# SamShue/EKF_SLAM

Measured on AMD Instinct MI355X. Metric: EKF update-steps/sec at N landmarks; HBM GB/s on (I−KH)P vs roofline, higher is better.
Workload: dtype f64

## Files before the change

### ekf_slam_amd/_lib.py

```python
import ctypes
import os
import subprocess

_HERE = os.path.dirname(os.path.abspath(__file__))
LIB_PATH = os.environ.get("EKF_LIB_PATH") or os.path.join(_HERE, "libekfslam.so")

EKF_OK = 0
EKF_ERR_INVALID_ARG, EKF_ERR_NO_DEVICE, EKF_ERR_HIP, EKF_ERR_CAPACITY = 1, 2, 3, 4
EKF_ERR_INDEX, EKF_ERR_LOOKUP, EKF_ERR_STATE, EKF_ERR_COMM = 5, 6, 7, 8
EKF_MODE_KNOWN, EKF_MODE_UC = 0, 1
EKF_COMM_ID_BYTES = 128
EKF_MERGE_BATCH_MAX = 32
EKF_STORE_F64, EKF_STORE_F32 = 0, 1
EKF_ARITH_F64, EKF_ARITH_F32, EKF_ARITH_SPLIT3 = 0, 1, 2
(EKF_KERNEL_DOWNDATE, EKF_KERNEL_GATHER, EKF_KERNEL_PREDICT, EKF_KERNEL_ASSOCIATE, EKF_KERNEL_APPEND,
 EKF_KERNEL_ROWPANEL, EKF_KERNEL_EXCHANGE, EKF_KERNEL_COMPACT, EKF_KERNEL_COUNT) = range(9)

_d = ctypes.c_double
_dp = ctypes.POINTER(ctypes.c_double)
_i32 = ctypes.c_int32
_i64 = ctypes.c_int64
_vp = ctypes.c_void_p


class EkfConfig(ctypes.Structure):
    _fields_ = [("C", _d), ("Rc", _d * 2), ("s_cost", _d), ("s_thresh", _d), ("w_pos", _d),
                ("capacity_landmarks", _i64), ("mode", _i32), ("storage", _i32), ("device", _i32),
                ("tile", _i32), ("rank", _i32), ("world", _i32), ("batch", _i32), ("async_flush", _i32), ("device_assoc", _i32),
                ("pass_direction", _i32), ("force_sharded", _i32), ("pass_arith", _i32), ("reserved", _i32 * 2)]


SIGNATURES = {
    "ekf_abi_version": (_i32, []),
    "ekf_status_string": (ctypes.c_char_p, [_i32]),
    "ekf_config_default": (_i32, [ctypes.POINTER(EkfConfig), _i32]),
    "ekf_create": (_i32, [ctypes.POINTER(EkfConfig), ctypes.POINTER(_vp)]),
    "ekf_destroy": (_i32, [_vp]),
    "ekf_last_error": (ctypes.c_char_p, [_vp]),
    "ekf_set_stream": (_i32, [_vp, _vp]),
    "ekf_sync": (_i32, [_vp]),
    "ekf_flush": (_i32, [_vp]),
    "ekf_pending": (_i32, [_vp, ctypes.POINTER(_i32)]),
    "ekf_set_params": (_i32, [_vp, _d, _dp, _d, _d, _d]),
    "ekf_predict": (_i32, [_vp, _dp]),
    "ekf_motion_model": (_i32, [_dp, _i64, _dp, _dp, _dp]),
    "ekf_append": (_i32, [_vp, _dp, _dp, _dp, _d]),
    "ekf_correct": (_i32, [_vp, _dp, _dp, _i64]),
    "ekf_associate": (_i32, [_vp, _dp, _dp, ctypes.POINTER(_i32), ctypes.POINTER(_i64), _dp, _dp]),
    "ekf_associate_begin": (_i32, [_vp, _dp, _dp, _i32]),
    "ekf_associate_finish": (_i32, [_vp, ctypes.POINTER(_i32), ctypes.POINTER(_i64), _dp, _dp]),
    "ekf_measure": (_i32, [_vp, _dp, _i64, _dp, _dp, _dp, _i64]),
    "ekf_comm_unique_id": (_i32, [ctypes.c_char_p]),
    "ekf_comm_init": (_i32, [_vp, ctypes.c_char_p]),
    "ekf_hint_next": (_i32, [_vp, _i64]),
    "ekf_correct_begin": (_i32, [_vp, _dp, _dp, _i64]),
    "ekf_correct_finish": (_i32, [_vp]),
    "ekf_prefetch_rows": (_i32, [_vp, ctypes.POINTER(_i64), _i32]),
    "ekf_prefetch_next": (_i32, [_vp, ctypes.POINTER(_i64), _i32]),
    "ekf_prefetch_begin": (_i32, [_vp, ctypes.POINTER(_i64), _i32]),
    "ekf_prefetch_finish": (_i32, [_vp]),
    "ekf_exchange_info": (_i32, [_vp, ctypes.POINTER(_vp), ctypes.POINTER(_vp), ctypes.POINTER(_i64),
                                 ctypes.POINTER(_i64)]),
    "ekf_exchange_set_buffers": (_i32, [_vp, _vp, _vp]),
    "ekf_exchange_local": (_i32, [ctypes.POINTER(_vp), _i32]),
    "ekf_exchange_set_hook": (_i32, [_vp, _vp, _vp]),
    "ekf_shard_owner": (_i32, [_i32, _i64, _i64]),
    "ekf_shard_slot": (_i64, [_i32, _i64, _i64]),
    "ekf_shard_panel_source": (_i32, [_i32, _i64, _i64, ctypes.POINTER(_i32), ctypes.POINTER(_i64)]),
    "ekf_num_landmarks": (_i32, [_vp, ctypes.POINTER(_i64)]),
    "ekf_get_x": (_i32, [_vp, _dp]),
    "ekf_set_x": (_i32, [_vp, _dp, _i64]),
    "ekf_get_s": (_i32, [_vp, _dp]),
    "ekf_set_s": (_i32, [_vp, _dp, _i64]),
    "ekf_remove_landmarks": (_i32, [_vp, ctypes.POINTER(_i64), _i64]),
    "ekf_constrain_landmarks": (_i32, [_vp, _i64, _i64, _dp, _dp]),
    "ekf_merge_landmarks": (_i32, [_vp, _i64, _i64, _dp]),
    "ekf_merge_landmarks_batch": (_i32, [_vp, ctypes.POINTER(_i64), ctypes.POINTER(_i64), _i64, _dp, _dp]),
    "ekf_landmark_distance": (_i32, [_vp, _i64, _i64, _dp, _dp, _dp, _dp]),
    "ekf_nearest_landmarks": (_i32, [_vp, _dp, _dp, ctypes.POINTER(_i64)]),
    "ekf_diag_poke_device_signature": (_i32, [_vp, _i64, _d]),
    "ekf_get_P": (_i32, [_vp, _dp]),
    "ekf_set_P": (_i32, [_vp, _dp, _i64]),
    "ekf_get_P_block": (_i32, [_vp, _i64, _i64, _i64, _i64, _dp]),
    "ekf_get_P_diag_blocks": (_i32, [_vp, _dp]),
    "ekf_get_Q": (_i32, [_vp, _dp]),
    "ekf_load_lowrank_state": (_i32, [_vp, _i64, _dp, _dp, _dp, _dp, _i64]),
    "ekf_checkpoint_save": (_i32, [_vp, ctypes.c_char_p]),
    "ekf_checkpoint_load": (_i32, [_vp, ctypes.c_char_p]),
    "ekf_P_digest": (_i32, [_vp, _dp]),
    "ekf_device_bytes": (_i32, [_vp, ctypes.POINTER(_i64)]),
    "ekf_kernel_timing_enable": (_i32, [_vp, _i32, _i32]),
    "ekf_kernel_timing_read": (_i32, [_vp, _i32, ctypes.POINTER(_i64), _dp]),
    "ekf_downdate_kernel_name": (ctypes.c_char_p, [_vp, ctypes.POINTER(_i32)]),
    "ekf_downdate_algorithmic_bytes": (_i32, [_vp, ctypes.POINTER(_i64)]),
}

_LIB = None


class EkfError(RuntimeError):
    def __init__(self, status, message):
        super().__init__("libekfslam status %d: %s" % (status, message))
        self.status = status


def build():
    subprocess.check_call(["make", "-s", "-C", os.path.join(_HERE, "csrc")])


def lib():
    global _LIB
    if _LIB is None:
        if not os.path.exists(LIB_PATH):
            raise ImportError("libekfslam.so is not built (%s); run __graft_entry__.build() or "
                              "`make -C ekf_slam_amd/csrc` -- there is no fallback path" % LIB_PATH)
        if os.environ.get("EKF_NO_TORCH", "0") != "1":
            try:
                import torch
            except ImportError:
                pass
        L = ctypes.CDLL(LIB_PATH)
        for name, (res, args) in SIGNATURES.items():
            fn = getattr(L, name)
            fn.restype = res
            fn.argtypes = args
        _LIB = L
    return _LIB

EXCHANGE_HOOK = ctypes.CFUNCTYPE(ctypes.c_int32, ctypes.c_void_p)
```

### ekf_slam_amd/csrc/gather.h

```cpp
#pragma once

constexpr int kGatherCols = 256;
constexpr int kGatherBlock = kGatherCols + 3 * 64;

__device__ __forceinline__ double lane_bcast(double v, int src) {
    const int lo = __builtin_amdgcn_readlane(__double2loint(v), src), hi = __builtin_amdgcn_readlane(__double2hiint(v), src);
    return __hiloint2double(hi, lo);
}
__device__ __forceinline__ double lane_gather(double v, int src) {
    const int lo = __builtin_amdgcn_ds_bpermute(src << 2, __double2loint(v)), hi = __builtin_amdgcn_ds_bpermute(src << 2, __double2hiint(v));
    return __hiloint2double(hi, lo);
}
__device__ __forceinline__ double lane_xor1(double v) {
    const int lo = __builtin_amdgcn_mov_dpp(__double2loint(v), 0xB1, 0xF, 0xF, true), hi = __builtin_amdgcn_mov_dpp(__double2hiint(v), 0xB1, 0xF, 0xF, true);
    return __hiloint2double(hi, lo);
}
__device__ __forceinline__ void wave_lds_sync() { asm volatile("s_waitcnt lgkmcnt(0)" ::: "memory"); }

constexpr int kFuseMaxRows = 48;
constexpr int kFuseElems = kFuseMaxRows * kFuseMaxRows / 256;

template <typename TS>
__device__ __forceinline__ void gather_decided_other(const DevState &st, const CorrectArgs &a, const DevLoopArgs &dl, int64_t Nd,
                                                     bool append) {
    __shared__ double oa_ll[kGatherCols / 64];
    __shared__ int oa_ix[kGatherCols / 64];
    const int tid = threadIdx.x;
    if (tid >= kGatherCols) return;
    const int cur = a.cur;
    const double *__restrict__ x = st.x[cur];
    const double *__restrict__ strip = st.strip[cur];
    const double *__restrict__ prr = st.prr[cur];
    double *__restrict__ x_nxt = st.x[cur ^ 1];
    double *__restrict__ strip_nxt = st.strip[cur ^ 1];
    double *__restrict__ prr_nxt = st.prr[cur ^ 1];
    const double *__restrict__ dg = st.diag[st.dcur];
    double *__restrict__ dgn = st.diag[st.dcur ^ 1];
    TS *__restrict__ tiles = (TS *)st.tiles;
    const int64_t ldm = st.ldm;
    const int64_t n_old = 2 * Nd, n_new = append ? n_old + 2 : n_old;
    const int64_t c = (int64_t)blockIdx.x * kGatherCols + tid;
    const bool live = c < n_new;
    double pose[3], pr[9];
#pragma unroll
    for (int i = 0; i < 3; ++i) pose[i] = x[i];
#pragma unroll
    for (int i = 0; i < 9; ++i) pr[i] = prr[i];
    double jxr[2][3];
    append_jxr(dl.u0, pose[2], jxr);
    double xn = 0.0, t0 = 0.0, t1 = 0.0, t2 = 0.0, dgc = 0.0, dgl = 0.0;
    if (c < n_old) {
        t0 = strip[c]; t1 = strip[ldm + c]; t2 = strip[2 * ldm + c];
        xn = x[3 + c];
        const double *__restrict__ d = dg + 3 * (c >> 1);
        if (c & 1) { dgl = d[1]; dgc = d[2]; } else dgc = d[0];
        if (append)
            for (int i = 0; i < 2; ++i)
                if (st.tm.mine((n_old + i) >> st.tm.shift, c >> st.tm.shift))
                    pmm_low_store<TS>(tiles, st.tm, n_old + i, c, append_row_entry(jxr, i, t0, t1, t2));
    } else if (live) {
        const int b = (int)(c - n_old);
        const volatile double *loc = dl.loc + 3 * (Nd - dl.loc_base);
        double cblk[3], iblk[3][2];
        append_blocks(jxr, pr, dl.u0, dl.u1, a.R00, a.R01, a.R10, a.R11, cblk, iblk);
        xn = loc[b];
        t0 = iblk[0][b]; t1 = iblk[1][b]; t2 = iblk[2][b];
        const bool own = st.tm.mine(n_old >> st.tm.shift, n_old >> st.tm.shift);
        if (b == 0) {
            dgc = cblk[0];
            if (own) pmm_low_store<TS>(tiles, st.tm, n_old, n_old, cblk[0]);
            st.s[Nd] = (double)(Nd + 1);
        } else {
            dgl = cblk[1]; dgc = cblk[2];
            if (own) { pmm_low_store<TS>(tiles, st.tm, n_old + 1, n_old, cblk[1]); pmm_low_store<TS>(tiles, st.tm, n_old + 1, n_old + 1, cblk[2]); }
        }
    }
    if (live) {
        x_nxt[3 + c] = xn;
        strip_nxt[c] = t0; strip_nxt[ldm + c] = t1; strip_nxt[2 * ldm + c] = t2;
        double *__restrict__ d = dgn + 3 * (c >> 1);
        if (c & 1) { d[1] = dgl; d[2] = dgc; } else d[0] = dgc;
    }
    if (c < st.tm.padded(n_new)) {
        const int64_t out_off = (int64_t)ring_slot(a.pstart, a.npend, st.pcap) * st.pair_stride;
        reinterpret_cast<double2 *>(st.Gp + out_off)[c] = make_double2(0.0, 0.0);
        reinterpret_cast<double2 *>(st.Kp + out_off)[c] = make_double2(0.0, 0.0);
        if (st.Gp32) {
            st.Gp32[out_off + c] = 0.0f; st.Gp32[out_off + ldm + c] = 0.0f;
            st.Kp32[out_off + c] = -0.0f; st.Kp32[out_off + ldm + c] = -0.0f;
        }
    }
    if (blockIdx.x == 0) {
        if (tid < 9) prr_nxt[tid] = prr[tid];
        if (tid < 3) x_nxt[tid] = x[tid];
        if (tid == 0) *dl.dn_out = n_new >> 1;
    }
    if (dl.parts_out == nullptr) return;
    const bool odd = (c & 1) != 0;
    const double xn_o = lane_xor1(xn), t0_o = lane_xor1(t0), t1_o = lane_xor1(t1), t2_o = lane_xor1(t2),
                 d10 = lane_xor1(dgl), d11 = lane_xor1(dgc);
    double ll = INFINITY;
    int64_t ix = INT64_MAX;
    if (live && !odd) {
        const int64_t k = c >> 1;
        double q[24];
#pragma unroll
        for (int i = 0; i < 9; ++i) q[i] = pr[i];
        q[9] = t0; q[10] = t0_o; q[11] = t1; q[12] = t1_o; q[13] = t2; q[14] = t2_o;
        q[15] = dgc; q[16] = d10; q[17] = d10; q[18] = d11;
        q[19] = pose[0]; q[20] = pose[1]; q[21] = pose[2];
        q[22] = xn; q[23] = xn_o;
        SmallSolve so;
        solve_small(q, dl.z0, dl.z1, dl.R00, dl.R01, dl.R10, dl.R11, so);
        const double n0 = so.nu[0], n1 = so.nu[1];
        const double pc = (n0 * so.Phi[0] + n1 * so.Phi[2]) * n0 + (n0 * so.Phi[1] + n1 * so.Phi[3]) * n1;
        const double sk = k == Nd ? (double)(Nd + 1) : st.s[k];
        const double d = dl.z2 - sk;
        const double sc = d * (1.0 / dl.s_cost) * d;
        const double like = (dl.w_pos != 0.0) ? (dl.w_pos * pc + sc) : sc;
        if (like <= dl.s_thresh) { ll = like; ix = k; }
    }
    wave_argmin_sparse(ll, ix);
    if ((tid & 63) == 0) { oa_ll[tid >> 6] = ll; oa_ix[tid >> 6] = ix == INT64_MAX ? -1 : (int)ix; }
    __syncthreads();
    if (tid < 64) {
        ll = tid < kGatherCols / 64 ? oa_ll[tid] : INFINITY;
        ix = (tid < kGatherCols / 64 && oa_ix[tid] >= 0) ? (int64_t)oa_ix[tid] : INT64_MAX;
        if (ix == INT64_MAX) ll = INFINITY;
        wave_argmin_sparse(ll, ix);
        if (tid == 0) store_partial(dl.parts_out + blockIdx.x, ll, ix == INT64_MAX ? -1 : (int)ix, dl.seq_out);
    }
}

template <typename TS, bool kSharded, bool kPredict, bool kFused = false, bool kDev = false, bool kDecide = false>
__global__ __launch_bounds__(kGatherBlock) void k_gather(DevState st, CorrectArgs a, PanelView pv, PredictArgs pa,
                                                         typename DevLoopParam<kDev>::type dl) {
    static_assert(!kDev || !kFused, "the device loop never drives the small-map fused form");
    static_assert(!kDecide || (kDev && !kSharded && !kPredict), "the device-decided branch: unsharded, predict carried out before");
    __shared__ double pss[24];
    __shared__ SmallSolve sol;
    __shared__ PredictSmall ps;
    __shared__ double pose_sh[3];
    __shared__ int diag_ready;
    __shared__ int staged_cnt;
    __shared__ double2 upatch[kMaxPending * 4];
    const int tid = threadIdx.x;
    const int role = __builtin_amdgcn_readfirstlane(tid >> 6);
    const int lane = tid & 63;
    const int cur = a.cur;
    const double *__restrict__ x = cur ? st.x[1] : st.x[0];
    const double *__restrict__ strip = cur ? st.strip[1] : st.strip[0];
    const double *__restrict__ prr_cur = cur ? st.prr[1] : st.prr[0];
    double *__restrict__ x_nxt = cur ? st.x[0] : st.x[1];
    double *__restrict__ strip_nxt = cur ? st.strip[0] : st.strip[1];
    double *__restrict__ prr_nxt = cur ? st.prr[0] : st.prr[1];
    const TS *__restrict__ tiles = (const TS *)st.tiles;
    int64_t j = a.j;
    const int64_t ldm = st.ldm;
    const int npend = a.npend, pstart = a.pstart;
    if constexpr (kDev) {
        double dll;
        int dix;
        reduce_partials_wave(dl.parts_in, dl.nblk_in, dl.seq_in, lane, dll, dix);
        dix = __builtin_amdgcn_readfirstlane(dix);
        if constexpr (kDecide) {
            const int64_t Nd = dl.n_known >= 0 ? dl.n_known : *dl.dn_in;
            a.n_mm = 2 * Nd;
            const bool stopped = *(volatile int32_t *)dl.abort == dl.scan_id;
            if (stopped || !(dix >= 0 && (int64_t)dix < Nd)) {
                int code = stopped ? -3 : dix;
                if (code == -1 && *(const volatile double *)(dl.loc + 3 * (Nd - dl.loc_base) + 2) != 1.0) {
                    code = -4;
                    if (blockIdx.x == 0 && tid == kGatherCols + 64) *(volatile int32_t *)dl.abort = dl.scan_id;
                }
                if (blockIdx.x == 0 && tid == kGatherCols + 128) store_partial(dl.rec, dll, code, dl.seq_rec);
                gather_decided_other<TS>(st, a, dl, Nd, code == -1);
                return;
            }
            if (blockIdx.x == 0 && tid == kGatherCols + 64) *dl.dn_out = Nd;
        }
        if (dix >= 0 && 2 * (int64_t)dix < a.n_mm) j = 2 * (int64_t)dix;
        if constexpr (kSharded) pv.Ij = j >> st.tm.shift;
        if (blockIdx.x == 0 && tid == kGatherCols + 128) store_partial(dl.rec, dll, dix, dl.seq_rec);
    }

    {
        const double *t_tiles = (const double *)st.tiles;
        asm volatile("" :: "s"(st.ldm), "s"(st.pair_stride), "s"(st.pcap), "s"(st.Gp), "s"(st.Kp), "s"(t_tiles), "s"(st.small),
                     "s"(st.tm.T), "s"(st.tm.shift), "s"(st.tm.world), "s"(st.tm.rank), "s"(a.j), "s"(a.n_mm), "s"(a.npend),
                     "s"(a.pstart));
    }
    const bool do_patch = !kSharded || !pv.patched;
#ifdef EKF_GATHER_STAMPS
    long long stamp[12]; int nst = 0;
#define EKF_STAMP() do { stamp[nst++] = clock64(); } while (0)
    EKF_STAMP();
#else
#define EKF_STAMP() do { } while (0)
#endif

    if (role >= 4) {
        double small_v = 0.0;
        if (role == 4) {
            const double *sp = prr_cur;
            if (lane < 9) sp = prr_cur + lane;
            else if (lane < 15) { const int t = (lane - 9) >> 1, b = (lane - 9) & 1; sp = strip + t * ldm + j + b; }
            else if (lane >= 19 && lane < 22) sp = x + (lane - 19);
            else if (lane >= 22 && lane < 24) sp = x + 3 + j + (lane - 22);
            small_v = *sp;
            if (lane == 24) { diag_ready = 0; staged_cnt = 0; }
        } else if (role == 5) {
            const int t = (lane >> 1) & 1, b = lane & 1;
            small_v = st.diag[st.dcur][3 * (j >> 1) + (t > b ? t : b) + (t > b ? b : t)];
        } else {
            small_v = x[lane < 3 ? lane : 3 + j + ((lane - 3) & 1)];
        }
        __builtin_amdgcn_sched_barrier(0);
        asm volatile("s_barrier" ::: "memory");
        EKF_STAMP();
        if (role == 4 && (lane < 15 || (lane >= 19 && lane < 24))) pss[lane] = small_v;
        if (role == 5 && lane < 4) pss[15 + lane] = small_v;
        EKF_STAMP();
        if (role == 5) {
            wave_lds_sync();
            if (lane == 0) *(volatile int *)&diag_ready = 1;
            EKF_STAMP();
        } else if (role == 6) {
            const double bx = lane_bcast(small_v, 0), by = lane_bcast(small_v, 1), bth = lane_bcast(small_v, 2),
                         blx = lane_bcast(small_v, 3), bly = lane_bcast(small_v, 4);
            if (lane == 0) {
                double pose[3] = { bx, by, bth };
                if (kPredict) {
                    const double2 sc2 = sincosd_ni(pose[2] + pa.u1);
                    const double sn2 = sc2.x, cs2 = sc2.y;
                    const double p0 = predict_pose_entry(pose, 0, pa.u0, pa.u1, sn2, cs2), p1 = predict_pose_entry(pose, 1, pa.u0, pa.u1, sn2, cs2),
                                 p2 = predict_pose_entry(pose, 2, pa.u0, pa.u1, sn2, cs2);
                    pose[0] = p0; pose[1] = p1; pose[2] = p2;
                }
                const double d0 = blx - pose[0], d1 = bly - pose[1];
                const double bearing = bearing_ni(d1, d0, pose[2]);
                const double sq = sqrt(d0 * d0 + d1 * d1);
                sol.nu[0] = a.z0 - sq;
                sol.nu[1] = a.z1 - bearing;
            }
        } else {
            double p[24];
#pragma unroll
            for (int i = 0; i < 24; ++i) p[i] = (i >= 15 && i < 19) ? 0.0 : lane_bcast(small_v, i);
            double fa = 0.0, fb = 0.0;
            double pose[3] = { p[19], p[20], p[21] };
            if (kPredict) {
                const double2 sc_l = sincosd_ni((lane & 1) ? pose[2] + pa.u1 : pose[2]);
                EKF_STAMP();
                const double sn = lane_bcast(sc_l.x, 0), cs = lane_bcast(sc_l.y, 0), sn2 = lane_bcast(sc_l.x, 1), cs2 = lane_bcast(sc_l.y, 1);
                double W[3];
                predict_common(pa.u0, pa.u1, sn, cs, fa, fb, W);
                const int ri = lane >= 6 ? 2 : lane >= 3 ? 1 : 0, rj = lane - 3 * ri;
                const int ei = ri > rj ? ri : rj, ej = ri > rj ? rj : ri;
                const int st_t = (lane - 9) >> 1, st_b = (lane - 9) & 1;
                const bool is_prr = lane < 9;
                const int g0 = is_prr ? ej : 9 + st_b, g1 = is_prr ? 3 + ej : 11 + st_b, g2 = is_prr ? 6 + ej : 13 + st_b;
                const double v0 = lane_gather(small_v, g0 & 63), v1 = lane_gather(small_v, g1 & 63), v2 = lane_gather(small_v, g2 & 63);
                const double cj[3] = { v0, v1, v2 };
                const double c2[3] = { p[2], p[5], p[8] };
                const double wi = EKF_SEL(ei == 0) ? W[0] : (EKF_SEL(ei == 1) ? W[1] : W[2]);
                const double wj = EKF_SEL(ej == 0) ? W[0] : (EKF_SEL(ej == 1) ? W[1] : W[2]);
                double e_prr, e_q;
                predict_prr_entry(ei, ej, cj, c2, fa, fb, wi, wj, pa.C, e_prr, e_q);
                double s0 = v0, s1 = v1;
                predict_strip(s0, s1, v2, fa, fb);
                const double e_strip = EKF_SEL(st_t == 0) ? s0 : (EKF_SEL(st_t == 1) ? s1 : v2);
                const double p0 = predict_pose_entry(pose, 0, pa.u0, pa.u1, sn2, cs2), p1 = predict_pose_entry(pose, 1, pa.u0, pa.u1, sn2, cs2),
                             p2 = predict_pose_entry(pose, 2, pa.u0, pa.u1, sn2, cs2);
                pose[0] = p0; pose[1] = p1; pose[2] = p2;
                EKF_STAMP();
                if (lane < 15) pss[lane] = EKF_SEL(is_prr) ? e_prr : e_strip;
                if (lane < 9) ps.Q[lane] = e_q;
                if (lane == 0) { ps.fa = fa; ps.fb = fb; }
            }
            if (lane < 3) pose_sh[lane] = lane == 0 ? pose[0] : lane == 1 ? pose[1] : pose[2];
            SmallSolve so;
            double sq;
            solve_hs(p[22] - pose[0], p[23] - pose[1], sq, so.Hs);
            EKF_STAMP();
            while (*(volatile int *)&diag_ready == 0) { }
            wave_lds_sync();
            const int ra = lane >= 5 ? 1 : 0;
            double hsel[5];
#pragma unroll
            for (int t = 0; t < 5; ++t) hsel[t] = ra ? so.Hs[1][t] : so.Hs[0][t];
            const double e_gs = solve_gs_entry(pss, hsel, lane < 10 ? lane - 5 * ra : 0);
            double GS[2][5];
#pragma unroll
            for (int i = 0; i < 10; ++i) GS[i / 5][i % 5] = lane_bcast(e_gs, i);
            double e_phi;
            {
                const int aa = (lane >> 1) & 1, bb = lane & 1;
                double gsel[5], hb[5];
#pragma unroll
                for (int t = 0; t < 5; ++t) { gsel[t] = aa ? GS[1][t] : GS[0][t]; hb[t] = bb ? so.Hs[1][t] : so.Hs[0][t]; }
                const double Rab = aa == 0 ? (bb == 0 ? a.R00 : a.R01) : (bb == 0 ? a.R10 : a.R11);
                e_phi = solve_phi_entry(gsel, hb, Rab);
            }
            const double phi[4] = { lane_bcast(e_phi, 0), lane_bcast(e_phi, 1), lane_bcast(e_phi, 2), lane_bcast(e_phi, 3) };
            ekfm::inv2(phi, so.Phi);
            EKF_STAMP();
#pragma unroll
            for (int b = 0; b < 3; ++b) {
                so.Gr[0][b] = GS[0][b]; so.Gr[1][b] = GS[1][b];
#pragma unroll
                for (int cc = 0; cc < 2; ++cc) so.Kr[b][cc] = solve_kr_entry(GS[0][b], GS[1][b], so.Phi[cc], so.Phi[2 + cc]);
            }
            if (lane == 0) {
#pragma unroll
                for (int i = 0; i < 10; ++i) sol.Hs[i / 5][i % 5] = so.Hs[i / 5][i % 5];
#pragma unroll
                for (int i = 0; i < 4; ++i) sol.Phi[i] = so.Phi[i];
#pragma unroll
                for (int i = 0; i < 6; ++i) { sol.Kr[i / 2][i % 2] = so.Kr[i / 2][i % 2]; sol.Gr[i / 3][i % 3] = so.Gr[i / 3][i % 3]; }
            }
        }
        __syncthreads();
        if (blockIdx.x == 0) {
            if (role == 4) {
                if (lane < 3) x_nxt[lane] = pose_sh[lane] + (sol.Kr[lane][0] * sol.nu[0] + sol.Kr[lane][1] * sol.nu[1]);
            } else if (role == 5) {
                if (lane < 9) {
                    const int r = lane / 3, b = lane - 3 * r;
                    const int rr = r > b ? r : b, bb = r > b ? b : r;
                    prr_nxt[3 * r + b] = pss[3 * rr + bb] - (sol.Kr[rr][0] * sol.Gr[0][bb] + sol.Kr[rr][1] * sol.Gr[1][bb]);
                }
            } else {
                if (lane < 6) { const int r = lane / 3, b = lane - 3 * r; st.small[3 * r + b] = sol.Gr[r][b]; }
                else if (lane < 12) { const int b = (lane - 6) >> 1, r = (lane - 6) & 1; st.small[6 + 2 * b + r] = sol.Kr[b][r]; }
#if !defined(EKF_GATHER_STAMPS) || EKF_GATHER_STAMPS < 2
                else if (kPredict && lane < 21) st.small[12 + (lane - 12)] = ps.Q[lane - 12];
#endif
            }
        }
#ifdef EKF_GATHER_STAMPS
        EKF_STAMP();
#if EKF_GATHER_STAMPS == 2
        if (blockIdx.x == 0 && tid == kGatherCols) for (int i = 0; i < 9; ++i) st.small[12 + i] = (double)(stamp[i] - stamp[0]);
#endif
#if EKF_GATHER_STAMPS == 3
        if (blockIdx.x == 0 && tid == kGatherCols + 64) for (int i = 0; i < 9; ++i) st.small[12 + i] = (double)(stamp[i] - stamp[0]);
#endif
#endif
        return;
    }

    const int64_t c = (int64_t)blockIdx.x * kGatherCols + tid;
    const bool live = c < a.n_mm;
    static_assert(kMaxPending * 4 == 2 * kGatherCols, "two uniform operands per column lane");
    auto load_up = [&](int e0) {
        const int e = (do_patch && e0 < 4 * npend) ? e0 : 0;
        const int i = e >> 2, which = e & 3;
        const double *base = (which < 2 ? st.Kp : st.Gp) + (int64_t)ring_slot(pstart, i, st.pcap) * st.pair_stride;
        return reinterpret_cast<const double2 *>(base)[j + (which & 1)];
    };
    const double2 up0 = load_up(tid), up1 = load_up(tid + kGatherCols);
    __builtin_amdgcn_sched_barrier(0);
    asm volatile("s_barrier" ::: "memory");
    EKF_STAMP();
    double m0 = 0.0, m1 = 0.0, s0 = 0.0, s1 = 0.0, s2 = 0.0, xc = 0.0;
    const bool rowpart = c <= j, colpart = c >= j + 2;
    if (live) {
        if (kSharded) { const double2 m = pv.at(st.tm, c); m0 = m.x; m1 = m.y; }
        else if (rowpart) {
            const int64_t m = st.tm.T - 1;
            const TS *__restrict__ tp = tiles + st.tm.tile_offset(j >> st.tm.shift, c >> st.tm.shift) + ((j & m) << st.tm.shift) + (c & m);
            m0 = (double)tp[0]; m1 = (double)tp[st.tm.T];
        }
        else if (colpart) pmm_low_pair<TS>(tiles, st.tm, c, j, m0, m1);
        else pmm_low_pair<TS>(tiles, st.tm, j + 1, j, m0, m1);
        s0 = strip[c]; s1 = strip[ldm + c]; s2 = strip[2 * ldm + c];
        xc = x[3 + c];
    }
    double dgc = 0.0, dgl = 0.0;
    if (live) {
        const double *__restrict__ dg = st.diag[st.dcur] + 3 * (c >> 1);
        if (c & 1) { dgl = dg[1]; dgc = dg[2]; } else dgc = dg[0];
    }
    __builtin_amdgcn_sched_barrier(0);
    EKF_STAMP();
    upatch[tid] = up0; upatch[tid + kGatherCols] = up1;
    wave_lds_sync();
    if ((tid & 63) == 0) atomicAdd(&staged_cnt, 1);
    while (*(volatile int *)&staged_cnt < 4) { }
    wave_lds_sync();
    EKF_STAMP();

    constexpr int kPre = 32;
    const int npre = do_patch ? (npend < kPre ? npend : kPre) : 0;
    const int64_t pad_cols = st.tm.padded(a.n_mm);
    const int64_t ps2 = st.pair_stride / 2;
    double2 pre[kPre];
    bool next_assoc = false;
    if constexpr (kDev) next_assoc = dl.parts_out != nullptr;
    {
        const uint32_t cc = (uint32_t)(c < pad_cols ? c : pad_cols - 1);
        const uint32_t krel = (uint32_t)((st.Kp - st.Gp) >> 1);
        const uint32_t lane_off = cc + (rowpart ? 0u : krel);
        const char *__restrict__ ub = reinterpret_cast<const char *>(st.Gp);
        const uint32_t lane_bytes = lane_off * 16u;
        const uint32_t step = (uint32_t)ps2, wrap = (uint32_t)st.pcap * step;
        uint32_t off = (uint32_t)pstart * step;
        int npre_ld = npre;
        asm volatile("" : "+s"(npre_ld));
#pragma unroll
        for (int g0 = 0; g0 < kPre; g0 += 8) {
            if (g0 < npre_ld) {
#pragma unroll
                for (int t = 0; t < 8; ++t) {
                    pre[g0 + t] = *reinterpret_cast<const double2 *>(ub + (uint64_t)off * 16u + lane_bytes);
                    if (g0 + t + 1 < npre) { off += step; if (off == wrap) off = 0; }
                }
            }
        }
    }


    if (live && do_patch) {
        if (rowpart) {
#pragma unroll
            for (int g0 = 0; g0 < kPre; g0 += 8)
                if (g0 < npre) {
                    double2 ua[8], ub[8];
#pragma unroll
                    for (int t = 0; t < 8; ++t) { ua[t] = upatch[4 * (g0 + t) + 0]; ub[t] = upatch[4 * (g0 + t) + 1]; }
#pragma unroll
                    for (int t = 0; t < 8; ++t) {
                        const double v0 = rank2_apply(m0, ua[t], pre[g0 + t]), v1 = rank2_apply(m1, ub[t], pre[g0 + t]);
                        m0 = g0 + t < npre ? v0 : m0; m1 = g0 + t < npre ? v1 : m1;
                    }
                }
            const double2 *__restrict__ gp = reinterpret_cast<const double2 *>(st.Gp) + c;
            int i = npre;
            for (; i + 8 <= npend; i += 8) {
                double2 g[8];
#pragma unroll
                for (int q = 0; q < 8; ++q) g[q] = gp[(int64_t)ring_slot(pstart, i + q, st.pcap) * ps2];
#pragma unroll
                for (int q = 0; q < 8; ++q) {
                    m0 = rank2_apply(m0, upatch[4 * (i + q) + 0], g[q]);
                    m1 = rank2_apply(m1, upatch[4 * (i + q) + 1], g[q]);
                }
            }
            for (; i < npend; ++i) {
                const double2 g = gp[(int64_t)ring_slot(pstart, i, st.pcap) * ps2];
                m0 = rank2_apply(m0, upatch[4 * i + 0], g);
                m1 = rank2_apply(m1, upatch[4 * i + 1], g);
            }
        } else if (colpart) {
#pragma unroll
            for (int g0 = 0; g0 < kPre; g0 += 8)
                if (g0 < npre) {
                    double2 ua[8], ub[8];
#pragma unroll
                    for (int t = 0; t < 8; ++t) { ua[t] = upatch[4 * (g0 + t) + 2]; ub[t] = upatch[4 * (g0 + t) + 3]; }
#pragma unroll
                    for (int t = 0; t < 8; ++t) {
                        const double v0 = rank2_apply(m0, pre[g0 + t], ua[t]), v1 = rank2_apply(m1, pre[g0 + t], ub[t]);
                        m0 = g0 + t < npre ? v0 : m0; m1 = g0 + t < npre ? v1 : m1;
                    }
                }
            const double2 *__restrict__ kp = reinterpret_cast<const double2 *>(st.Kp) + c;
            int i = npre;
            for (; i + 8 <= npend; i += 8) {
                double2 k[8];
#pragma unroll
                for (int q = 0; q < 8; ++q) k[q] = kp[(int64_t)ring_slot(pstart, i + q, st.pcap) * ps2];
#pragma unroll
                for (int q = 0; q < 8; ++q) {
                    m0 = rank2_apply(m0, k[q], upatch[4 * (i + q) + 2]);
                    m1 = rank2_apply(m1, k[q], upatch[4 * (i + q) + 3]);
                }
            }
            for (; i < npend; ++i) {
                const double2 k = kp[(int64_t)ring_slot(pstart, i, st.pcap) * ps2];
                m0 = rank2_apply(m0, k, upatch[4 * i + 2]);
                m1 = rank2_apply(m1, k, upatch[4 * i + 3]);
            }
        } else {
            for (int i = 0; i < npend; ++i) {
                m0 = rank2_apply(m0, upatch[4 * i + 1], upatch[4 * i + 2]);
                m1 = rank2_apply(m1, upatch[4 * i + 1], upatch[4 * i + 3]);
            }
        }
    }
    {
        const double dgl_p = lane_xor1(dgl);
        if (c == j) { m0 = dgc; m1 = dgl_p; }
        else if (c == j + 1) { m0 = dgl; m1 = dgc; }
    }
    EKF_STAMP();
    __syncthreads();
    EKF_STAMP();

    const int64_t pad_end = st.tm.padded(a.n_mm);
    const int64_t out_off = (int64_t)ring_slot(pstart, npend, st.pcap) * st.pair_stride;
    double2 *__restrict__ Gout = reinterpret_cast<double2 *>(st.Gp + out_off);
    double2 *__restrict__ Kout = reinterpret_cast<double2 *>(st.Kp + out_off);
    double g[2] = { 0.0, 0.0 }, k0 = 0.0, k1 = 0.0;
    double xn = 0.0, t0 = 0.0, t1 = 0.0, t2 = 0.0;
    if (live) {
        if (kPredict) predict_strip(s0, s1, s2, ps.fa, ps.fb);
        for (int r = 0; r < 2; ++r)
            g[r] = sol.Hs[r][0] * s0 + sol.Hs[r][1] * s1 + sol.Hs[r][2] * s2 + sol.Hs[r][3] * m0 + sol.Hs[r][4] * m1;
        k0 = g[0] * sol.Phi[0] + g[1] * sol.Phi[2];
        k1 = g[0] * sol.Phi[1] + g[1] * sol.Phi[3];
        if (!kFused) {
            Gout[c] = make_double2(g[0], g[1]);
            Kout[c] = make_double2(k0, k1);
            if (st.Gp32) {
                st.Gp32[out_off + c] = (float)g[0]; st.Gp32[out_off + ldm + c] = (float)g[1];
                st.Kp32[out_off + c] = -(float)k0; st.Kp32[out_off + ldm + c] = -(float)k1;
            }
        }
        xn = xc + (k0 * sol.nu[0] + k1 * sol.nu[1]);
        t0 = s0 - (sol.Kr[0][0] * g[0] + sol.Kr[0][1] * g[1]);
        t1 = s1 - (sol.Kr[1][0] * g[0] + sol.Kr[1][1] * g[1]);
        t2 = s2 - (sol.Kr[2][0] * g[0] + sol.Kr[2][1] * g[1]);
        x_nxt[3 + c] = xn;
        double *__restrict__ sn = strip_nxt;
        sn[c] = t0;
        sn[ldm + c] = t1;
        sn[2 * ldm + c] = t2;
    } else if (c < pad_end && !kFused) {
        Gout[c] = make_double2(0.0, 0.0);
        Kout[c] = make_double2(0.0, 0.0);
        if (st.Gp32) {
            st.Gp32[out_off + c] = 0.0f; st.Gp32[out_off + ldm + c] = 0.0f;
            st.Kp32[out_off + c] = -0.0f; st.Kp32[out_off + ldm + c] = -0.0f;
        }
    }
    double ndc, ndl;
    {
        const double2 kn = make_double2(k0, k1), gn = make_double2(g[0], g[1]);
        const double2 gl = make_double2(lane_xor1(gn.x), lane_xor1(gn.y));
        ndc = rank2_apply(dgc, kn, gn);
        ndl = rank2_apply(dgl, kn, gl);
        if (live) {
            double *__restrict__ dn = st.diag[st.dcur ^ 1] + 3 * (c >> 1);
            if (c & 1) { dn[1] = ndl; dn[2] = ndc; } else dn[0] = ndc;
        }
    }
    if (kFused) {
        upatch[tid] = make_double2(k0, k1);
        upatch[kGatherCols + tid] = make_double2(g[0], g[1]);
        __syncthreads();
        {
            TS *__restrict__ tw = (TS *)st.tiles;
            const int sh = st.tm.shift, msk = st.tm.T - 1;
            const unsigned n = (unsigned)a.n_mm, total = n * n;
            TS *ptr[kFuseElems];
            double val[kFuseElems];
            unsigned rr[kFuseElems], cq[kFuseElems];
#pragma unroll
            for (int q = 0; q < kFuseElems; ++q) {
                const unsigned e = (unsigned)tid + 256u * q;
                const unsigned r = e / n, cx = e - r * n;
                const bool stored = e < total && (r >> sh) >= (cx >> sh);
                rr[q] = stored ? r : 0u; cq[q] = stored ? cx : 0u;
                ptr[q] = stored ? tw + st.tm.tile_offset(r >> sh, cx >> sh) + ((r & msk) << sh) + (cx & msk) : nullptr;
                val[q] = stored ? (double)*ptr[q] : 0.0;
            }
#pragma unroll
            for (int q = 0; q < kFuseElems; ++q)
                if (ptr[q]) *ptr[q] = (TS)rank2_apply(val[q], upatch[rr[q]], upatch[kGatherCols + cq[q]]);
        }
    }
    if constexpr (kDev) {
        if (next_assoc) {
            __shared__ double na_ll[kGatherCols / 64];
            __shared__ int na_ix[kGatherCols / 64];
            const bool odd = (c & 1) != 0;
            const double dcc = ndc, dlo = ndl;
            const double xn_o = lane_xor1(xn), t0_o = lane_xor1(t0), t1_o = lane_xor1(t1), t2_o = lane_xor1(t2),
                         d10 = lane_xor1(dlo), d11 = lane_xor1(dcc);
            double ll = INFINITY;
            int64_t ix = INT64_MAX;
            if (live && !odd) {
                const int64_t k = c >> 1;
                double q[24];
#pragma unroll
                for (int r = 0; r < 3; ++r)
#pragma unroll
                    for (int b = 0; b < 3; ++b) {
                        const int rr = r > b ? r : b, bb = r > b ? b : r;
                        q[3 * r + b] = pss[3 * rr + bb] - (sol.Kr[rr][0] * sol.Gr[0][bb] + sol.Kr[rr][1] * sol.Gr[1][bb]);
                    }
                q[9] = t0; q[10] = t0_o; q[11] = t1; q[12] = t1_o; q[13] = t2; q[14] = t2_o;
                q[15] = dcc; q[16] = d10; q[17] = d10; q[18] = d11;
#pragma unroll
                for (int l = 0; l < 3; ++l)
                    q[19 + l] = pose_sh[l] + (sol.Kr[l][0] * sol.nu[0] + sol.Kr[l][1] * sol.nu[1]);
                q[22] = xn; q[23] = xn_o;
                SmallSolve so2;
                solve_small(q, dl.z0, dl.z1, dl.R00, dl.R01, dl.R10, dl.R11, so2);
                const double n0 = so2.nu[0], n1 = so2.nu[1];
                const double pc = (n0 * so2.Phi[0] + n1 * so2.Phi[2]) * n0 + (n0 * so2.Phi[1] + n1 * so2.Phi[3]) * n1;
                const double d = dl.z2 - st.s[k];
                const double sc = d * (1.0 / dl.s_cost) * d;
                const double like = (dl.w_pos != 0.0) ? (dl.w_pos * pc + sc) : sc;
                if (like <= dl.s_thresh) { ll = like; ix = k; }
            }
            wave_argmin_sparse(ll, ix);
            if ((tid & 63) == 0) { na_ll[tid >> 6] = ll; na_ix[tid >> 6] = ix == INT64_MAX ? -1 : (int)ix; }
            __syncthreads();
            if (tid < 64) {
                ll = tid < kGatherCols / 64 ? na_ll[tid] : INFINITY;
                ix = (tid < kGatherCols / 64 && na_ix[tid] >= 0) ? (int64_t)na_ix[tid] : INT64_MAX;
                if (ix == INT64_MAX) ll = INFINITY;
                wave_argmin_sparse(ll, ix);
                if (tid == 0) store_partial(dl.parts_out + blockIdx.x, ll, ix == INT64_MAX ? -1 : (int)ix, dl.seq_out);
            }
        }
    }
#ifdef EKF_GATHER_STAMPS
    EKF_STAMP();
    __syncthreads();
#if EKF_GATHER_STAMPS == 1
    if (c == 0) for (int i = 0; i < 7; ++i) st.small[12 + i] = (double)(stamp[i] - stamp[0]);
#endif
#endif
#undef EKF_STAMP
}
```

### ekf_slam_amd/csrc/host/lifecycle.h

```cpp
#pragma once
namespace {
int32_t create_state(ekf_handle *h) {
    const int64_t ldm = h->st.ldm;
    for (int b = 0; b < 2; ++b) {
        HIPCHK(h, dalloc(h, &h->st.x[b], (size_t)(3 + ldm)));
        HIPCHK(h, dalloc(h, &h->st.prr[b], 16));
        HIPCHK(h, dalloc(h, &h->st.strip[b], (size_t)(3 * ldm)));
        HIPCHK(h, dalloc(h, &h->st.diag[b], (size_t)(3 * h->cap)));
    }
    h->st.dcur = 0;
    HIPCHK(h, dalloc(h, &h->st.s, (size_t)h->cap));
    HIPCHK(h, dalloc(h, &h->st.small, 32));
    HIPCHK(h, dalloc(h, &h->d_digest, kDigestDoubles));
    HIPCHK(h, dalloc(h, &h->d_csmall, 16));
    HIPCHK(h, halloc(h, &h->h_small, 32 * sizeof(double), hipHostMallocDefault));
    const double prr0[9] = { 0.1, 0, 0, 0, 0.1, 0, 0, 0, 0.1 };
    HIPCHK(h, hipMemcpy(h->st.prr[0], prr0, sizeof prr0, hipMemcpyHostToDevice));
    h->cur = 0;
    h->N = 0;
    return EKF_OK;
}
}

extern "C" {
int32_t ekf_create(const ekf_config *cfg, ekf_handle **out) {
    if (!cfg || !out) return EKF_ERR_INVALID_ARG;
    *out = nullptr;
    const int32_t T = cfg->tile == 0 ? (cfg->storage == EKF_STORE_F32 ? 256 : 128) : cfg->tile;
    const int32_t world = cfg->world <= 0 ? 1 : cfg->world;
    if (!(T == 16 || T == 32 || T == 64 || T == 128 || (T == 256 && cfg->storage == EKF_STORE_F32))) return EKF_ERR_INVALID_ARG;
    if (cfg->capacity_landmarks < 1 || cfg->rank < 0 || cfg->rank >= world) return EKF_ERR_INVALID_ARG;
    if (cfg->storage != EKF_STORE_F64 && cfg->storage != EKF_STORE_F32) return EKF_ERR_INVALID_ARG;
    if (cfg->mode != EKF_MODE_KNOWN && cfg->mode != EKF_MODE_UC) return EKF_ERR_INVALID_ARG;
    if (cfg->batch < 0 || cfg->batch > 64) return EKF_ERR_INVALID_ARG;
    if (cfg->mode == EKF_MODE_UC && cfg->device_assoc == 4 && (world > 1 || cfg->force_sharded)) return EKF_ERR_INVALID_ARG;
    if (cfg->pass_arith != EKF_ARITH_F64 &&
        !((cfg->pass_arith == EKF_ARITH_F32 || cfg->pass_arith == EKF_ARITH_SPLIT3) && cfg->storage == EKF_STORE_F32 && T == 256))
        return EKF_ERR_INVALID_ARG;
    int ndev = 0;
    if (hipGetDeviceCount(&ndev) != hipSuccess || ndev <= 0 || cfg->device < 0 || cfg->device >= ndev)
        return EKF_ERR_NO_DEVICE;

    ekf_handle *h = new (std::nothrow) ekf_handle();
    if (!h) return EKF_ERR_INVALID_ARG;
    h->cfg = *cfg;
    h->cfg.world = world;
    h->cfg.tile = T;
    h->T = T;
    h->cap = cfg->capacity_landmarks;
    h->storage = cfg->storage;
    *out = h;

    HIPCHK(h, hipSetDevice(cfg->device));
    hipDeviceProp_t prop = {};
    if (cfg->async_flush != 0 || cfg->pass_arith != EKF_ARITH_F64) HIPCHK(h, hipGetDeviceProperties(&prop, cfg->device));
    {
        int lo = 0, hi = 0;
        HIPCHK(h, hipDeviceGetStreamPriorityRange(&lo, &hi));
        HIPCHK(h, hipStreamCreateWithPriority(&h->own_stream, hipStreamNonBlocking, hi));
    }
    h->stream = h->own_stream;
    const int64_t nt_cap = ekf_tiles_for(2 * h->cap, T);
    h->st.ldm = nt_cap * T;
    h->st.tm = ekf_make_tilemap(T, world, cfg->rank);
    h->work_cap = h->st.tm.slots_for_rows(nt_cap);

    TRY(create_state(h));
    TRY(create_passes(h, prop));
    TRY(create_worklists(h));
    TRY(create_assoc(h));
    TRY(create_exchange(h));
    TRY(create_decided(h));
    HIPCHK(h, hipDeviceSynchronize());
    return EKF_OK;
}

int32_t ekf_destroy(ekf_handle *h) {
    if (!h) return EKF_OK;
    hipSetDevice(h->cfg.device);
    if (h->stream) hipStreamSynchronize(h->stream);
    if (h->comm && g_rccl.CommDestroy) g_rccl.CommDestroy(h->comm);
    for (hipStream_t s : { h->flush_stream, h->xchg_stream }) if (s) { hipStreamSynchronize(s); hipStreamDestroy(s); }
    for (hipEvent_t e : h->events) hipEventDestroy(e);
    for (auto &t : h->timers) for (hipEvent_t e : t.ev) hipEventDestroy(e);
    for (void *p : h->allocs) hipFree(p);
    for (void *p : h->pinned) hipHostFree(p);
    if (h->own_stream) hipStreamDestroy(h->own_stream);
    delete h;
    return EKF_OK;
}

int32_t ekf_kernel_timing_enable(ekf_handle *h, int32_t which, int32_t on) {
    if (!h || which < 0 || which >= EKF_KERNEL_COUNT) return fail(h, EKF_ERR_INVALID_ARG, "kernel_timing_enable: bad kernel id");
    TRY(use_device(h));
    HIPCHK(h, hipStreamSynchronize(h->stream));
    KernelTimer &t = h->timers[which];
    if (on) {
        const size_t reserve = on > 512 ? (size_t)on : 512;
        while (t.ev.size() < 2 * reserve) {
            hipEvent_t e;
            HIPCHK(h, hipEventCreate(&e));
            t.ev.push_back(e);
        }
    }
    t.enabled = on != 0;
    t.used = 0;
    return EKF_OK;
}

int32_t ekf_kernel_timing_read(ekf_handle *h, int32_t which, int64_t *launches, double *total_ms) {
    if (!h || which < 0 || which >= EKF_KERNEL_COUNT || !launches || !total_ms)
        return fail(h, EKF_ERR_INVALID_ARG, "kernel_timing_read: bad argument");
    TRY(use_device(h));
    HIPCHK(h, hipStreamSynchronize(h->stream));
    if (h->flush_stream) HIPCHK(h, hipStreamSynchronize(h->flush_stream));
    KernelTimer &t = h->timers[which];
    double tot = 0.0;
    for (size_t i = 0; i + 1 < t.used; i += 2) {
        float ms = 0.f;
        HIPCHK(h, hipEventElapsedTime(&ms, t.ev[i], t.ev[i + 1]));
        tot += ms;
    }
    *launches = (int64_t)(t.used / 2);
    *total_ms = tot;
    t.used = 0;
    return EKF_OK;
}
}
```

### ekf_slam_amd/csrc/host/passes.h

```cpp
#pragma once
namespace {
int32_t refresh_work(ekf_handle *h) {
    const int64_t nt = ekf_tiles_for(2 * n_hi(h), h->T);
    if (nt == h->ws[h->ws_cur].rows) return EKF_OK;
    const int32_t to = h->ws_pass == h->ws_cur ? h->ws_cur ^ 1 : h->ws_cur;
    ekf_handle::WorkSet &ws = h->ws[to];
    const size_t b_work = (size_t)h->work_cap * sizeof(int2), b_xcd = 8 * b_work, b_segs = (size_t)h->segs_cap * sizeof(int4);
    if (!h->wl_stage) h->wl_stage_bytes = b_work + b_xcd + b_segs;
    int32_t rc = stage_alloc(h, &h->wl_stage, h->wl_stage_bytes, &h->ev_wl);
    if (!rc) rc = stage_wait(h, h->ev_wl, h->wl_busy);
    if (rc) return rc;
    int2 *w = reinterpret_cast<int2 *>(h->wl_stage);
    int2 *flat = reinterpret_cast<int2 *>(h->wl_stage + b_work);
    int4 *segs = reinterpret_cast<int4 *>(h->wl_stage + b_work + b_xcd);
    size_t nw = 0;
    REQUIRE(h, h->st.tm.slots_for_rows(nt) <= h->work_cap, EKF_ERR_STATE, "work list overflow");
    for (int64_t I = 0; I < nt; ++I)
        for (int64_t J = 0; J <= I; ++J)
            if (h->st.tm.mine(I, J)) w[nw++] = make_int2((int)I, (int)J);
    if (nw) HIPCHK(h, hipMemcpyAsync(ws.work, w, nw * sizeof(int2), hipMemcpyHostToDevice, h->stream));
    ws.nwork = (int64_t)nw;
    ws.rows = nt;

    static const int S = std::max(1, ekf_tune_int("EKF_SUPERTILE", 8));
    struct Super { int64_t si, sj; std::vector<int2> tiles; };
    std::vector<Super> supers;
    const int64_t ns = (nt + S - 1) / S;
    for (int64_t si = 0; si < ns; ++si)
        for (int64_t sj = 0; sj <= si; ++sj) {
            Super sp; sp.si = si; sp.sj = sj;
            for (int64_t I = si * S; I < nt && I < (si + 1) * S; ++I)
                for (int64_t J = sj * S; J <= I && J < (sj + 1) * S; ++J)
                    if (h->st.tm.mine(I, J)) sp.tiles.push_back(make_int2((int)I, (int)J));
            if (!sp.tiles.empty()) supers.push_back(std::move(sp));
        }
    static const int order = ekf_tune_int("EKF_XCD_ORDER", 1);
    std::vector<int2> stream[8];
    if (order == 0) {
        std::stable_sort(supers.begin(), supers.end(), [](const Super &a, const Super &b) { return a.tiles.size() > b.tiles.size(); });
        for (const Super &sp : supers) {
            int best = 0;
            for (int x = 1; x < 8; ++x) if (stream[x].size() < stream[best].size()) best = x;
            stream[best].insert(stream[best].end(), sp.tiles.begin(), sp.tiles.end());
        }
    } else {
        std::vector<int2> flat_order;
        flat_order.reserve(nw);
        for (const Super &sp : supers) flat_order.insert(flat_order.end(), sp.tiles.begin(), sp.tiles.end());
        const size_t tot = flat_order.size();
        for (int x = 0; x < 8; ++x)
            stream[x].assign(flat_order.begin() + (tot * x) / 8, flat_order.begin() + (tot * (x + 1)) / 8);
    }
    size_t len = 0;
    for (int x = 0; x < 8; ++x) len = std::max(len, stream[x].size());
    REQUIRE(h, (int64_t)(8 * len) <= 8 * h->work_cap, EKF_ERR_STATE, "XCD work list overflow");
    std::fill(flat, flat + 8 * len, make_int2(-1, -1));
    for (int x = 0; x < 8; ++x) std::copy(stream[x].begin(), stream[x].end(), flat + x * len);
    if (len) HIPCHK(h, hipMemcpyAsync(ws.xcd, flat, 8 * len * sizeof(int2), hipMemcpyHostToDevice, h->stream));
    ws.xcd_len = (int64_t)len;
    if (ws.segs) {
        std::vector<int4> sg;
        const int64_t nsegs = ekf_pipe32::build_strip_segments(h->st.tm, nt, sg);
        REQUIRE(h, (int64_t)sg.size() <= h->segs_cap, EKF_ERR_STATE, "strip work list overflow");
        if (!sg.empty()) {
            std::copy(sg.begin(), sg.end(), segs);
            HIPCHK(h, hipMemcpyAsync(ws.segs, segs, sg.size() * sizeof(int4), hipMemcpyHostToDevice, h->stream));
        }
        ws.nsegs = nsegs;
        ws.cols = nt * h->T;
    }
    TRY(stage_uploaded(h, h->ev_wl, h->wl_busy));
    h->ws_cur = to;
    h->ws_unordered = true;
    return EKF_OK;
}

const PassAux *pass_aux(const ekf_handle *h, const ekf_handle::WorkSet &ws, PassAux &out) {
    if (!ws.segs) return nullptr;
    out = h->aux;
    out.segs = ws.segs; out.nsegs = ws.nsegs; out.cols = ws.cols;
    return &out;
}

PassJob pass_job(const ekf_handle *h, const ekf_handle::WorkSet &ws, void *dst, PassAux &ax) {
    PassJob job = {};
    job.dst = dst;
    job.work = ws.work; job.nwork = ws.nwork; job.work_xcd = ws.xcd; job.xcd_len = ws.xcd_len;
    job.pstart = h->pstart; job.npairs = h->npend;
    job.grid_cap = h->grid_cap; job.arith = h->cfg.pass_arith;
    job.aux = pass_aux(h, ws, ax);
    return job;
}

int32_t create_worklists(ekf_handle *h) {
    for (auto &ws : h->ws) {
        if (h->cfg.pass_arith != EKF_ARITH_F64) HIPCHK(h, dalloc(h, &ws.segs, (size_t)h->segs_cap));
        HIPCHK(h, dalloc(h, &ws.work, (size_t)h->work_cap));
        HIPCHK(h, dalloc(h, &ws.xcd, (size_t)h->work_cap * 8));
    }
    return EKF_OK;
}

int32_t retire_inflight(ekf_handle *h) {
    if (!h->inflight) return EKF_OK;
    if (h->appended_inflight) {
        if (!h->ev_rows) HIPCHK(h, new_event(h, &h->ev_rows));
        HIPCHK(h, hipEventRecord(h->ev_rows, h->stream));
        HIPCHK(h, hipStreamWaitEvent(h->flush_stream, h->ev_rows, 0));
        if (decided_mode(h)) {
            const int64_t *hi = unsettled(h) > 0 ? h->d_nring + h->nrow % ekf_handle::kNRing : nullptr;
            HIPCHK(h, launch_copy_rows_dev(h->st.tm, h->tilebuf[h->base], h->tilebuf[h->base ^ 1], 2 * h->inflight_N, 2 * n_hi(h), h->inflight_dn,
                                           hi, h->storage, h->flush_stream));
        } else
            HIPCHK(h, launch_copy_rows(h->st.tm, h->tilebuf[h->base], h->tilebuf[h->base ^ 1], 2 * h->inflight_N, 2 * h->N, h->storage, h->flush_stream));
        HIPCHK(h, hipEventRecord(h->ev_flushed, h->flush_stream));
        h->appended_inflight = false;
    }
    HIPCHK(h, hipStreamWaitEvent(h->stream, h->ev_flushed, 0));
    h->ws_pass = -1;
    h->base ^= 1;
    h->st.tiles = h->tilebuf[h->base];
    h->pstart = (h->pstart + h->nfrozen) % h->st.pcap;
    h->npend -= h->nfrozen;
    h->nfrozen = 0;
    h->inflight = false;
    tiles_changed(h);
    return EKF_OK;
}

void next_pass_direction(ekf_handle *h) {
    const int force = h->cfg.pass_direction == 1 ? 0 : h->cfg.pass_direction == 2 ? 1 : -1;
    constexpr int64_t kCacheBytes = 256ll << 20;
    const int64_t nt = ekf_tiles_for(2 * n_hi(h), h->T);
    const int64_t store = nt * (nt + 1) / 2 / std::max(1, h->cfg.world) * (int64_t)h->T * h->T * (h->storage == EKF_STORE_F64 ? 8 : 4);
    const bool alternate = force >= 0 ? force != 0 : store > kCacheBytes;
    h->st.tm.reverse = alternate ? (h->st.tm.reverse ^ 1) : 0;
}

int32_t flush_pending(ekf_handle *h, bool batch_done = false) {
    TRY(retire_inflight(h));
    if (h->npend == 0) return EKF_OK;
    TRY(refresh_work(h));
    next_pass_direction(h);
    bool extracted = false;
    const int64_t hint = h->hint_idx;
    bool pn = false, pn_side = false;
    if (batch_done && !h->pn_idx.empty()) {
        if (h->sharded && !h->pending && h->pn_N == h->N && (h->comm || h->xhook)) {
            const int32_t m = (int32_t)h->pn_idx.size();
            const int64_t slab = slab_for(h, n_mm(h));
            TIMED(h, EKF_KERNEL_ROWPANEL, launch_rowpanel_next(h->st, h->pn_idx.data(), m, n_mm(h), h->pstart, h->npend, h->send, slab, h->storage,
                  h->stream));
            tiles_changed(h);
            h->pf_idx = h->pn_idx; h->pf_m = m; h->pf_slab = slab; h->pf_N = h->N;
            h->x_count = (int64_t)m * slab;
            static const int pn_side_stream = ekf_tune_int("EKF_PN_SIDE_STREAM", 0);
            if (h->comm) {
                pn_side = pn_side_stream != 0;
                if (pn_side && !h->xchg_stream) {
                    HIPCHK(h, hipStreamCreateWithFlags(&h->xchg_stream, hipStreamNonBlocking));
                    HIPCHK(h, new_event(h, &h->ev_pn_ready));
                    HIPCHK(h, new_event(h, &h->ev_pn_done));
                }
                if (pn_side) {
                    HIPCHK(h, hipEventRecord(h->ev_pn_ready, h->stream));
                    HIPCHK(h, hipStreamWaitEvent(h->xchg_stream, h->ev_pn_ready, 0));
                }
                const hipStream_t xs = pn_side ? h->xchg_stream : h->stream;
                const int r = g_rccl.AllGather(h->send, h->recv, (size_t)h->x_count,  8, h->comm, xs);
                if (r != 0) return fail(h, EKF_ERR_COMM, g_rccl.GetErrorString(r));
                HIPCHK(h, store_panels(h, xs));
                if (pn_side) HIPCHK(h, hipEventRecord(h->ev_pn_done, h->xchg_stream));
            } else {
                TRY(exchange_bracket(h, 2));
                HIPCHK(h, store_panels(h, h->stream));
            }
            pn = true;
        }
        drop_announced(h);
    }
    {
        NextRow nx = { -1, nullptr };
        if (h->sharded && h->npend == 1 && !h->pending && hint >= 0 && hint < h->N) {
            nx.j = 2 * hint;
            nx.send = corr_send(h, slab_for(h, n_mm(h)));
        }
        TimedLaunch tl(h, EKF_KERNEL_DOWNDATE);
        const ekf_handle::WorkSet &ws = h->ws[h->ws_cur];
        PassAux ax;
        PassJob job = pass_job(h, ws, h->st.tiles, ax);
        job.nx = nx.j >= 0 ? &nx : nullptr;
        HIPCHK(h, launch_downdate(h->st, job, h->storage, h->stream, h->dd_kernel, &extracted));
        h->dd_pairs = h->npend;
    }
    h->npend = 0;
    h->pstart = 0;
    h->pf_valid = pn;
    if (pn_side) HIPCHK(h, hipStreamWaitEvent(h->stream, h->ev_pn_done, 0));
    h->nx_valid = extracted && !pn;
    if (extracted) { h->nx_idx = hint; h->nx_N = h->N; }
    return EKF_OK;
}

int32_t batch_complete(ekf_handle *h) {
    if (!h->async_flush) return flush_pending(h,  true);
    HIPCHK(h, hipEventRecord(h->ev_pairs, h->stream));
    h->ws_unordered = false;
    TRY(retire_inflight(h));
    TRY(refresh_work(h));
    HIPCHK(h, hipStreamWaitEvent(h->flush_stream, h->ev_pairs, 0));
    if (h->ws_unordered) HIPCHK(h, hipStreamWaitEvent(h->flush_stream, h->ev_wl, 0));
    {
        TimedLaunch tl(h, EKF_KERNEL_DOWNDATE, h->flush_stream);
        next_pass_direction(h);
        const ekf_handle::WorkSet &ws = h->ws[h->ws_cur];
        PassAux ax;
        HIPCHK(h, launch_downdate(h->st, pass_job(h, ws, h->tilebuf[h->base ^ 1], ax), h->storage, h->flush_stream, h->dd_kernel));
        h->dd_pairs = h->npend;
    }
    HIPCHK(h, hipEventRecord(h->ev_flushed, h->flush_stream));
    h->nfrozen = h->npend;
    h->inflight = true;
    h->ws_pass = h->ws_cur;
    h->inflight_N = h->N;
    h->inflight_dn = unsettled(h) > 0 ? h->d_nring + h->nrow % ekf_handle::kNRing : nullptr;
    h->appended_inflight = false;
    return EKF_OK;
}

int32_t create_passes(ekf_handle *h, const hipDeviceProp_t &prop) {
    const ekf_config &cfg = h->cfg;
    const int32_t T = h->T;
    const int64_t ldm = h->st.ldm, slots = h->work_cap, nt_cap = ldm / T;
    char *tiles = nullptr;
    HIPCHK(h, dalloc(h, &tiles, (size_t)slots * T * T * elt_size(h)));
    h->st.tiles = tiles;
    h->tilebuf[0] = tiles;
    h->async_flush = cfg.async_flush != 0;
    if (h->async_flush) {
        char *tiles2 = nullptr;
        HIPCHK(h, dalloc(h, &tiles2, (size_t)slots * T * T * elt_size(h)));
        h->tilebuf[1] = tiles2;
        int reserve = ekf_tune_int("EKF_ASYNC_RESERVE_CUS", cfg.pass_arith == EKF_ARITH_SPLIT3 ? 64 : 32);
        const int ncu = prop.multiProcessorCount;
        if (reserve > 0 && ncu == 256) {
            if (reserve > 128) reserve = 128;
            uint32_t mask[8];
            for (int w = 0; w < 8; ++w) mask[w] = 0xffffffffu;
            int taken = 0;
            for (int b = 0; b < 16 && taken < reserve; ++b)
                for (int a = 0; a < 8 && taken < reserve; ++a) {
                    const int bit = 32 * a + 8 * (b & 3) + ((a + (b >> 2)) & 7);
                    if (mask[bit >> 5] & (1u << (bit & 31))) { mask[bit >> 5] &= ~(1u << (bit & 31)); ++taken; }
                }
            HIPCHK(h, hipExtStreamCreateWithCUMask(&h->flush_stream, 8, mask));
            h->flush_cus = ncu - taken;
        } else {
            int lo = 0, hi = 0;
            HIPCHK(h, hipDeviceGetStreamPriorityRange(&lo, &hi));
            HIPCHK(h, hipStreamCreateWithPriority(&h->flush_stream, hipStreamNonBlocking, lo));
        }
        HIPCHK(h, new_event(h, &h->ev_pairs));
        HIPCHK(h, new_event(h, &h->ev_flushed));
    }
    h->batch = cfg.batch < 1 ? 1 : cfg.batch;
    h->cfg.batch = h->batch;
    h->st.pair_stride = 2 * ldm;
    h->st.pcap = h->async_flush ? 2 * h->batch : h->batch;
    HIPCHK(h, dalloc(h, &h->st.Gp, (size_t)(2 * ldm) * h->st.pcap * 2));
    h->st.Kp = h->st.Gp + (size_t)(2 * ldm) * h->st.pcap;
    h->st.Gp32 = nullptr; h->st.Kp32 = nullptr;
    if (cfg.pass_arith != EKF_ARITH_F64) {
        HIPCHK(h, dalloc(h, &h->st.Gp32, (size_t)(2 * ldm) * h->st.pcap * 2));
        h->st.Kp32 = h->st.Gp32 + (size_t)(2 * ldm) * h->st.pcap;
        h->aux.grid = prop.multiProcessorCount > 0 ? prop.multiProcessorCount : 256;
        if (h->flush_cus > 0) h->aux.grid = h->flush_cus;
        h->aux.grid -= h->aux.grid % 8;
        if (h->aux.grid < 8) h->aux.grid = 8;
        const int64_t ranges = (2 * nt_cap + ekf_pipe32::kSeg * cfg.world - 1) / (ekf_pipe32::kSeg * cfg.world);
        h->segs_cap = 4 * slots + (2 * nt_cap * ranges + 8) * ekf_pipe32::kSeg;
        float *dump = nullptr;
        HIPCHK(h, dalloc(h, &dump, (size_t)h->aux.grid * ekf_pipe32::kDumpFloats));
        h->aux.dump = dump;
        if (cfg.pass_arith == EKF_ARITH_SPLIT3) {
            HIPCHK(h, dalloc(h, &h->aux.Kb3, pass_split_plane_elems(ldm)));
            HIPCHK(h, dalloc(h, &h->aux.Gb3, pass_split_plane_elems(ldm)));
        }
    }
    h->grid_cap = ekf_tune_int("EKF_DOWNDATE_GRID", 0);
    return EKF_OK;
}
}
```

### ekf_slam_amd/csrc/kernels.h

```cpp
#pragma once
#include <hip/hip_runtime.h>
#include <stdint.h>

#include "layout.h"

#ifdef EKF_TUNING
#include <stdlib.h>
inline int ekf_tune_int(const char *name, int dflt) { const char *v = getenv(name); return v ? atoi(v) : dflt; }
#else
constexpr int ekf_tune_int(const char *, int dflt) { return dflt; }
#endif

struct DevState {
    double *x[2];
    double *prr[2];
    double *strip[2];
    void   *tiles;
    double *s;
    double *Gp;
    double *Kp;
    float  *Gp32;
    float  *Kp32;
    int64_t pair_stride;
    int32_t pcap;
    double *small;
    int64_t ldm;
    TileMap tm;
    double *diag[2];
    int32_t dcur;
};

struct PredictArgs {
    double u0, u1, C;
    int64_t n_mm;
    int32_t cur;
};
hipError_t launch_predict(const DevState &st, const PredictArgs &a, int storage, hipStream_t s);

struct AssocHostPartial;

struct DevLoopArgs {
    const AssocHostPartial *parts_in;
    AssocHostPartial *rec;
    AssocHostPartial *parts_out;
    int32_t nblk_in, seq_in;
    int32_t seq_rec, seq_out;
    double z0, z1, z2;
    double R00, R01, R10, R11;
    double s_cost, s_thresh, w_pos;
    const int64_t *dn_in;
    int64_t *dn_out;
    int64_t n_known;
    const double *loc;
    int64_t loc_base;
    double u0, u1;
    int32_t *abort;
    int32_t scan_id;
};

struct AppendArgs {
    double u0, u1;
    double R00, R01, R10, R11;
    double pos0, pos1, signature;
    int64_t N;
    int32_t cur;
};
hipError_t launch_append(const DevState &st, const AppendArgs &a, int storage, hipStream_t s, const DevLoopArgs *dl = nullptr,
                         const PredictArgs *fused_predict = nullptr);

struct CorrectArgs {
    double z0, z1;
    double R00, R01, R10, R11;
    int64_t j;
    int64_t n_mm;
    int32_t cur;
    int32_t npend;
    int32_t pstart;
};
hipError_t launch_gather(const DevState &st, const CorrectArgs &a, const PredictArgs *fused_predict, int storage,
                         hipStream_t s, bool fuse_downdate);
int gather_fuse_max_rows();
hipError_t launch_gather_devloop(const DevState &st, const CorrectArgs &a, const PredictArgs *fused_predict, const DevLoopArgs &dl,
                                 int storage, hipStream_t s);
int64_t gather_workgroups(const DevState &st, int64_t n_mm);
hipError_t launch_gather_decided(const DevState &st, const CorrectArgs &a, const DevLoopArgs &dl, int storage, hipStream_t s);

hipError_t launch_rowpanel(const DevState &st, int64_t j, int64_t n_mm, int pstart, int npend, double *send, int storage,
                           hipStream_t s);
hipError_t launch_rowpanel_dev(const DevState &st, int64_t j, int64_t n_mm, int pstart, int npend, double *send, int storage,
                               hipStream_t s, const DevLoopArgs &dl);
struct RowList { int32_t m; int32_t j[64]; };
hipError_t launch_rowpanel_base(const DevState &st, const int64_t *idx, int m, int64_t n_mm, double *send, int64_t slab,
                                int storage, hipStream_t s);
hipError_t launch_rowpanel_next(const DevState &st, const int64_t *idx, int m, int64_t n_mm, int pstart, int npend, double *send,
                                int64_t slab, int storage, hipStream_t s);
hipError_t launch_gather_sharded(const DevState &st, const CorrectArgs &a, const PredictArgs *fused_predict, const double *recv,
                                 int64_t rank_stride, int64_t offset, bool patched, int storage, hipStream_t s,
                                 const DevLoopArgs *dl = nullptr);

struct AssocArgs {
    double z0, z1, z2;
    double R00, R01, R10, R11;
    double s_cost, s_thresh, w_pos;
    int64_t N;
    int32_t cur;
    int32_t npend;
    int32_t pstart;
    int32_t own_only;
    const int64_t *dN;
};

struct AssocDecision {
    int64_t index;
    int32_t is_new;
    int32_t seq;
    double  min_ll;
};

struct alignas(16) AssocHostPartial {
    double  min_ll;
    int32_t index;
    int32_t tag;
};
#if defined(__HIPCC__)
__host__ __device__
#endif
inline uint32_t assoc_part_mix(uint32_t ll_lo, uint32_t ll_hi, uint32_t index) {
    uint32_t m = ll_lo * 0x9E3779B1u ^ (ll_hi + 0x7F4A7C15u) * 0x85EBCA6Bu ^ (index + 0x165667B1u) * 0xC2B2AE35u;
    m ^= m >> 15; m *= 0x2C1B3C6Du; m ^= m >> 13;
    return m;
}

constexpr int kAssocBlock = 256;

hipError_t launch_associate(const DevState &st, const AssocArgs &a, double *pos_cost, double *sig_cost,
                            AssocDecision *partial, int *ticket, AssocDecision *decision, AssocHostPartial *host_partials, int seq,
                            double *cand, int storage, hipStream_t s, const PredictArgs *fused_predict = nullptr);
hipError_t launch_associate_devn(const DevState &st, const AssocArgs &a, AssocHostPartial *host_partials, int seq, int storage,
                                 hipStream_t s, const PredictArgs *fused_predict);
hipError_t launch_assoc_merge(const DevState &st, const double *recv, int world, int64_t count, int64_t N, bool want_costs,
                              double *pos_cost, AssocDecision *decision, AssocDecision *host_decision, int seq, hipStream_t s);

struct NextRow { int64_t j; double *send; };
struct PassAux {
    const int4 *segs;
    int64_t nsegs;
    float *dump;
    int grid;
    int64_t cols;
    uint16_t *Kb3, *Gb3;
};
size_t pass_split_plane_elems(int64_t ldm);
struct PassJob {
    void *dst;
    const int2 *work;
    int64_t nwork;
    const int2 *work_xcd;
    int64_t xcd_len;
    int pstart, npairs;
    int grid_cap;
    int arith;
    const PassAux *aux;
    const NextRow *nx;
};
hipError_t launch_downdate(const DevState &st, const PassJob &job, int storage, hipStream_t s, char *kname, bool *extracted = nullptr);
hipError_t launch_copy_rows(const TileMap &tm, const void *src, void *dst, int64_t r0, int64_t r1, int storage, hipStream_t s);
hipError_t launch_copy_rows_dev(const TileMap &tm, const void *src, void *dst, int64_t r0, int64_t r1, const int64_t *n_lo,
                                const int64_t *n_hi, int storage, hipStream_t s);

hipError_t launch_compact_tiles(const TileMap &tm, const void *src, void *dst, const int2 *work, int64_t ntiles, const int32_t *src_of,
                                int storage, hipStream_t s);
hipError_t launch_compact_state(const DevState &st, int cur, const int32_t *src_of, int64_t N_old, double *s_out, hipStream_t s);
struct ConstrainArgs {
    double d0, d1;
    double R00, R01, R10, R11;
    int64_t ai, aj;
    int64_t n_mm;
    int32_t cur;
    int32_t npend;
    int32_t pstart;
};
hipError_t launch_constrain_probe(const DevState &st, int cur, int64_t ai, int64_t aj, double *out, int storage, hipStream_t s);
hipError_t launch_gather_constrain(const DevState &st, const ConstrainArgs &a, int storage, hipStream_t s);
constexpr int kConstrainRecordDoubles = 8;
hipError_t launch_gather_constrain_chain(const DevState &st, const ConstrainArgs &a, double *rec, int storage, hipStream_t s);
hipError_t launch_merge_pass(const DevState &st, void *dst, const int2 *work, int64_t ntiles, const int32_t *src_of, int npairs,
                             int storage, hipStream_t s, char *kname);
struct alignas(16) NearestEntry { double d2; int64_t partner; };
hipError_t launch_nearest(const DevState &st, int cur, int64_t N, const double R[4], NearestEntry *out, int storage, hipStream_t s);

hipError_t launch_unpack_dense(const DevState &st, int cur, int64_t n_mm, double *dense, int storage, hipStream_t s);
hipError_t launch_pack_dense(const DevState &st, int cur, int64_t n_mm, const double *dense, int storage, hipStream_t s);
hipError_t launch_get_block(const DevState &st, int cur, int64_t r0, int64_t c0, int64_t nr, int64_t nc,
                            double *out, int storage, hipStream_t s);
hipError_t launch_get_diag_blocks(const DevState &st, int cur, int64_t N, double *out, int storage, hipStream_t s);
hipError_t launch_lowrank(const DevState &st, int cur, int64_t n_mm, const int2 *work, int64_t nwork, const double *d,
                          const double *U, int64_t k, int storage, hipStream_t s);
constexpr int kDigestGrid = 2048;
constexpr int kDigestDoubles = 4 + 3 * kDigestGrid;
hipError_t launch_digest(const DevState &st, int cur, int64_t n_mm, const int2 *work, int64_t nwork, double *out,
                         int storage, hipStream_t s);
```

### ekf_slam_amd/csrc/launch/steps.h

```cpp
#pragma once

hipError_t launch_predict(const DevState &st, const PredictArgs &a, int, hipStream_t s) {
    static const int force = ekf_tune_int("EKF_PREDICT_MFMA", -1);
    const bool mfma = force >= 0 ? force != 0 : a.n_mm >= 2048;
    if (mfma) {
        const int64_t nslices = (a.n_mm + 15) / 16;
        int64_t grid = cdiv(nslices > 0 ? nslices : 1, 4);
        if (grid > 1024) grid = 1024;
        hipLaunchKernelGGL(k_predict_mfma, dim3((unsigned)grid), dim3(kBlock), 0, s, st, a);
        return hipGetLastError();
    }
    const int64_t grid = cdiv(a.n_mm > 0 ? a.n_mm : 1, kBlock);
    hipLaunchKernelGGL(k_predict, dim3((unsigned)grid), dim3(kBlock), 0, s, st, a);
    return hipGetLastError();
}

hipError_t launch_append(const DevState &st, const AppendArgs &a, int storage, hipStream_t s, const DevLoopArgs *dlp,
                         const PredictArgs *fused_predict) {
    const int64_t n_mm = 2 * a.N;
    const int64_t grid = cdiv(n_mm > 0 ? n_mm : 1, kBlock);
    const DevLoopArgs dl = dlp ? *dlp : DevLoopArgs{};
    const PredictArgs pa = predict_or_none(fused_predict);
    return with_storage(storage, [&](auto ts) { with_bool(fused_predict != nullptr, [&](auto pred) {
        hipLaunchKernelGGL((k_append<decltype(ts), decltype(pred)::value>), dim3((unsigned)grid), dim3(kBlock), 0, s, st, a, dl, pa);
    }); });
}

int64_t gather_workgroups(const DevState &st, int64_t n_mm) { return cdiv(ekf_tiles_for(n_mm, st.tm.T) * st.tm.T, kGatherCols); }
int gather_fuse_max_rows() { return kFuseMaxRows; }

namespace {
template <bool kSharded, bool kFused, bool kDev, bool kDecide>
hipError_t gather_form(const DevState &st, const CorrectArgs &a, const PredictArgs *fused_predict, const PanelView &pv,
                       const DevLoopArgs *dl, int storage, hipStream_t s) {
    typename DevLoopParam<kDev>::type dla{};
    if constexpr (kDev) {
        if (!dl->parts_in || !dl->rec || dl->nblk_in < 1 || a.n_mm < 2) return hipErrorInvalidValue;
        dla = *dl;
    }
    const int64_t grid = gather_workgroups(st, a.n_mm);
    const PredictArgs pa = predict_or_none(fused_predict);
    return with_storage(storage, [&](auto ts) {
        auto launch = [&](auto pred) {
            hipLaunchKernelGGL((k_gather<decltype(ts), kSharded, decltype(pred)::value, kFused, kDev, kDecide>), dim3((unsigned)grid),
                               dim3(kGatherBlock), 0, s, st, a, pv, pa, dla);
        };
        if constexpr (kDecide) launch(std::false_type{});
        else with_bool(fused_predict != nullptr, launch);
    });
}
}

hipError_t launch_gather(const DevState &st, const CorrectArgs &a, const PredictArgs *fused_predict, int storage,
                         hipStream_t s, bool fuse_downdate) {
    if (!fuse_downdate) return gather_form<false, false, false, false>(st, a, fused_predict, PanelView{}, nullptr, storage, s);
    if (a.n_mm > kFuseMaxRows || gather_workgroups(st, a.n_mm) != 1) return hipErrorInvalidValue;
    return gather_form<false, true, false, false>(st, a, fused_predict, PanelView{}, nullptr, storage, s);
}

hipError_t launch_gather_devloop(const DevState &st, const CorrectArgs &a, const PredictArgs *fused_predict, const DevLoopArgs &dl,
                                 int storage, hipStream_t s) {
    return gather_form<false, false, true, false>(st, a, fused_predict, PanelView{}, &dl, storage, s);
}

hipError_t launch_gather_decided(const DevState &st, const CorrectArgs &a, const DevLoopArgs &dl, int storage, hipStream_t s) {
    if (!dl.dn_out || !dl.loc || !dl.abort || (dl.n_known < 0 && !dl.dn_in)) return hipErrorInvalidValue;
    return gather_form<false, false, true, true>(st, a, nullptr, PanelView{}, &dl, storage, s);
}

hipError_t launch_gather_sharded(const DevState &st, const CorrectArgs &a, const PredictArgs *fused_predict, const double *recv,
                                 int64_t rank_stride, int64_t offset, bool patched, int storage, hipStream_t s, const DevLoopArgs *dl) {
    const PanelView pv = { recv, rank_stride, offset,  a.j >> st.tm.shift, patched ? 1 : 0 };
    return dl ? gather_form<true, false, true, false>(st, a, fused_predict, pv, dl, storage, s)
              : gather_form<true, false, false, false>(st, a, fused_predict, pv, nullptr, storage, s);
}

hipError_t launch_rowpanel(const DevState &st, int64_t j, int64_t n_mm, int pstart, int npend, double *send, int storage,
                           hipStream_t s) {
    const int64_t nloc = rowpanel_local_chunks(st.tm, j, n_mm);
    if (nloc == 0) return hipSuccess;
    const int64_t grid = cdiv(nloc * st.tm.T, kBlock);
    return with_storage(storage, [&](auto ts) {
        hipLaunchKernelGGL(k_rowpanel<decltype(ts)>, dim3((unsigned)grid), dim3(kBlock), 0, s, st, j, n_mm, pstart, npend, send, nloc, NoDevLoop{});
    });
}

hipError_t launch_rowpanel_dev(const DevState &st, int64_t j, int64_t n_mm, int pstart, int npend, double *send, int storage,
                               hipStream_t s, const DevLoopArgs &dl) {
    if (!dl.parts_in || dl.nblk_in < 1) return hipErrorInvalidValue;
    const int64_t nt = ekf_tiles_for(n_mm, st.tm.T);
    const int64_t most = (nt + st.tm.world - 1) / st.tm.world;
    const int64_t grid = cdiv(most * st.tm.T, kBlock);
    return with_storage(storage, [&](auto ts) {
        hipLaunchKernelGGL((k_rowpanel<decltype(ts), true>), dim3((unsigned)grid), dim3(kBlock), 0, s, st, j, n_mm, pstart, npend, send, (int64_t)0, dl);
    });
}

namespace {
template <typename Launch>
hipError_t rowpanel_prefetch(const DevState &st, const int64_t *idx, int m, int64_t n_mm, bool args_ok, Launch &&launch) {
    if (m <= 0) return hipSuccess;
    if (m > 64 || !args_ok) return hipErrorInvalidValue;
    RowList rows;
    rows.m = m;
    for (int q = 0; q < m; ++q) rows.j[q] = (int32_t)(2 * idx[q]);
    const int64_t nt = st.tm.tiles_for(n_mm);
    const int64_t max_chunks = (nt + st.tm.world - 1) / st.tm.world;
    if (max_chunks == 0) return hipSuccess;
    return launch(rows, dim3((unsigned)cdiv(max_chunks * st.tm.T, kBlock), (unsigned)m));
}
}

hipError_t launch_rowpanel_base(const DevState &st, const int64_t *idx, int m, int64_t n_mm, double *send, int64_t slab,
                                int storage, hipStream_t s) {
    return rowpanel_prefetch(st, idx, m, n_mm, true, [&](const RowList &rows, dim3 grid) { return with_storage(storage, [&](auto ts) {
        hipLaunchKernelGGL(k_rowpanel_base<decltype(ts)>, grid, dim3(kBlock), 0, s, st, rows, n_mm, send, slab);
    }); });
}

hipError_t launch_rowpanel_next(const DevState &st, const int64_t *idx, int m, int64_t n_mm, int pstart, int npend, double *send,
                                int64_t slab, int storage, hipStream_t s) {
    const bool ring_ok = npend >= 0 && npend <= kMaxPending;
    return rowpanel_prefetch(st, idx, m, n_mm, ring_ok, [&](const RowList &rows, dim3 grid) { return with_storage(storage, [&](auto ts) {
        hipLaunchKernelGGL(k_rowpanel_next<decltype(ts)>, grid, dim3(kBlock), 0, s, st, rows, n_mm, pstart, npend, send, slab);
    }); });
}

namespace {
template <bool kDevN>
hipError_t associate_form(const DevState &st, const AssocArgs &a, double *pos_cost, double *sig_cost, AssocDecision *partial, int *ticket,
                          AssocDecision *decision, AssocHostPartial *host_partials, int seq, double *cand, int storage, hipStream_t s,
                          const PredictArgs *fused_predict) {
    const int64_t grid = cdiv(a.N > 0 ? a.N : 1, kAssocBlock);
    const PredictArgs pa = predict_or_none(fused_predict);
    return with_storage(storage, [&](auto ts) { with_bool(fused_predict != nullptr, [&](auto pred) {
        hipLaunchKernelGGL((k_associate<decltype(ts), decltype(pred)::value, kDevN>), dim3((unsigned)grid), dim3(kAssocBlock), 0, s, st, a, pos_cost,
                           sig_cost, partial, ticket, decision, host_partials, seq, cand, pa);
    }); });
}
}

hipError_t launch_associate(const DevState &st, const AssocArgs &a, double *pos_cost, double *sig_cost,
                            AssocDecision *partial, int *ticket, AssocDecision *decision, AssocHostPartial *host_partials, int seq,
                            double *cand, int storage, hipStream_t s, const PredictArgs *fused_predict) {
    return associate_form<false>(st, a, pos_cost, sig_cost, partial, ticket, decision, host_partials, seq, cand, storage, s, fused_predict);
}

hipError_t launch_associate_devn(const DevState &st, const AssocArgs &a, AssocHostPartial *host_partials, int seq, int storage,
                                 hipStream_t s, const PredictArgs *fused_predict) {
    if (!host_partials) return hipErrorInvalidValue;
    return associate_form<true>(st, a, nullptr, nullptr, nullptr, nullptr, nullptr, host_partials, seq, nullptr, storage, s, fused_predict);
}

hipError_t launch_assoc_merge(const DevState &st, const double *recv, int world, int64_t count, int64_t N, bool want_costs,
                              double *pos_cost, AssocDecision *decision, AssocDecision *host_decision, int seq, hipStream_t s) {
    int64_t grid = want_costs ? cdiv(N > 0 ? N : 1, kBlock) : 1;
    if (grid > 1024) grid = 1024;
    hipLaunchKernelGGL(k_assoc_merge, dim3((unsigned)grid), dim3(kBlock), 0, s, st.tm, recv, world, count, N, want_costs ? 1 : 0,
                       pos_cost, decision, host_decision, seq);
    return hipGetLastError();
}
```

### include/ekfslam.h

```cpp
#ifndef EKFSLAM_H
#define EKFSLAM_H

#include <stdint.h>

#ifdef __cplusplus
extern "C" {
#endif

#define EKF_ABI_VERSION 1

enum {
    EKF_OK = 0,
    EKF_ERR_INVALID_ARG = 1,
    EKF_ERR_NO_DEVICE = 2,
    EKF_ERR_HIP = 3,
    EKF_ERR_CAPACITY = 4,
    EKF_ERR_INDEX = 5,
    EKF_ERR_LOOKUP = 6,
    EKF_ERR_STATE = 7,
    EKF_ERR_COMM = 8
};

enum { EKF_MODE_KNOWN = 0,
       EKF_MODE_UC = 1 };

enum { EKF_STORE_F64 = 0,
       EKF_STORE_F32 = 1 };
enum { EKF_ARITH_F64 = 0,
       EKF_ARITH_F32 = 1,
       EKF_ARITH_SPLIT3 = 2 };

typedef struct ekf_config {
    double  C;
    double  Rc[2];
    double  s_cost;
    double  s_thresh;
    double  w_pos;
    int64_t capacity_landmarks;
    int32_t mode;
    int32_t storage;
    int32_t device;
    int32_t tile;
    int32_t rank;
    int32_t world;
    int32_t batch;
    int32_t async_flush;
    int32_t device_assoc;
    int32_t pass_direction;
    int32_t force_sharded;
    int32_t pass_arith;
    int32_t reserved[2];
} ekf_config;

typedef struct ekf_handle ekf_handle;

int32_t     ekf_abi_version(void);
const char *ekf_status_string(int32_t status);
int32_t     ekf_config_default(ekf_config *cfg, int32_t mode);

int32_t     ekf_create(const ekf_config *cfg, ekf_handle **out);
int32_t     ekf_destroy(ekf_handle *h);
const char *ekf_last_error(const ekf_handle *h);
int32_t     ekf_set_stream(ekf_handle *h, void *hip_stream);
int32_t     ekf_sync(ekf_handle *h);
int32_t     ekf_flush(ekf_handle *h);
int32_t     ekf_pending(ekf_handle *h, int32_t *npending);
int32_t     ekf_set_params(ekf_handle *h, double C, const double Rc[2], double s_cost, double s_thresh, double w_pos);

int32_t ekf_predict(ekf_handle *h, const double u[2]);

int32_t ekf_motion_model(const double *x, int64_t n, const double u[2], double *x_new, double *F);

int32_t ekf_append(ekf_handle *h, const double u[2], const double R[4], const double pos[2], double signature);

int32_t ekf_correct(ekf_handle *h, const double z[2], const double R[4], int64_t idx);

int32_t ekf_associate(ekf_handle *h, const double z[3], const double R[4], int32_t *is_new, int64_t *idx,
                      double *pos_cost, double *sig_cost);
int32_t ekf_associate_begin(ekf_handle *h, const double z[3], const double R[4], int32_t want_costs);
int32_t ekf_associate_finish(ekf_handle *h, int32_t *is_new, int64_t *idx, double *pos_cost, double *sig_cost);

int32_t ekf_measure(ekf_handle *h, const double *observed_LL, int64_t m, const double u[2],
                    const double *lm_index, const double *lm_loc, int64_t L);

int32_t ekf_hint_next(ekf_handle *h, int64_t idx);

typedef struct ekf_comm_id { char internal[128]; } ekf_comm_id;
int32_t ekf_comm_unique_id(ekf_comm_id *id);
int32_t ekf_comm_init(ekf_handle *h, const ekf_comm_id *id);
int32_t ekf_exchange_set_hook(ekf_handle *h, int32_t (*hook)(void *ctx), void *ctx);
int32_t ekf_correct_begin(ekf_handle *h, const double z[2], const double R[4], int64_t idx);
int32_t ekf_correct_finish(ekf_handle *h);
int32_t ekf_prefetch_rows(ekf_handle *h, const int64_t *idx, int32_t m);
int32_t ekf_prefetch_next(ekf_handle *h, const int64_t *idx, int32_t m);
int32_t ekf_prefetch_begin(ekf_handle *h, const int64_t *idx, int32_t m);
int32_t ekf_prefetch_finish(ekf_handle *h);
int32_t ekf_exchange_info(ekf_handle *h, void **send, void **recv, int64_t *count, int64_t *count_capacity);
int32_t ekf_exchange_set_buffers(ekf_handle *h, void *send, void *recv);
int32_t ekf_exchange_local(ekf_handle **shards, int32_t world);
int32_t ekf_shard_owner(int32_t world, int64_t I, int64_t J);
int64_t ekf_shard_slot(int32_t world, int64_t I, int64_t J);
int32_t ekf_shard_panel_source(int32_t world, int64_t tile_row_j, int64_t chunk, int32_t *owner, int64_t *local_chunk);

int32_t ekf_num_landmarks(ekf_handle *h, int64_t *N);
int32_t ekf_get_x(ekf_handle *h, double *x );
int32_t ekf_set_x(ekf_handle *h, const double *x, int64_t n);
int32_t ekf_get_s(ekf_handle *h, double *s );
int32_t ekf_set_s(ekf_handle *h, const double *s, int64_t N);
int32_t ekf_remove_landmarks(ekf_handle *h, const int64_t *idx, int64_t m);
int32_t ekf_constrain_landmarks(ekf_handle *h, int64_t i, int64_t j, const double delta[2], const double R[4]);
int32_t ekf_merge_landmarks(ekf_handle *h, int64_t keep, int64_t drop, const double R[4]);
#define EKF_MERGE_BATCH_MAX 32
int32_t ekf_merge_landmarks_batch(ekf_handle *h, const int64_t *keep, const int64_t *drop, int64_t m,
                                  const double R[4] ,
                                  double *d2 );
int32_t ekf_landmark_distance(ekf_handle *h, int64_t i, int64_t j, const double delta[2], const double R[4],
                              double *d2, double S[4] );
int32_t ekf_nearest_landmarks(ekf_handle *h, const double R[4] ,
                              double *d2 , int64_t *partner );
int32_t ekf_diag_poke_device_signature(ekf_handle *h, int64_t idx, double value);
int32_t ekf_get_P(ekf_handle *h, double *P);
int32_t ekf_set_P(ekf_handle *h, const double *P, int64_t n);
int32_t ekf_get_P_block(ekf_handle *h, int64_t r0, int64_t c0, int64_t nr, int64_t nc, double *out);
int32_t ekf_get_P_diag_blocks(ekf_handle *h, double *out );
int32_t ekf_get_Q(ekf_handle *h, double Q[9]);
int32_t ekf_load_lowrank_state(ekf_handle *h, int64_t N, const double *x, const double *s,
                               const double *d, const double *U, int64_t k);
int32_t ekf_P_digest(ekf_handle *h, double out[3]);
int32_t ekf_device_bytes(ekf_handle *h, int64_t *bytes);

int32_t ekf_checkpoint_save(ekf_handle *h, const char *path);
int32_t ekf_checkpoint_load(ekf_handle *h, const char *path);

enum { EKF_KERNEL_DOWNDATE = 0, EKF_KERNEL_GATHER = 1, EKF_KERNEL_PREDICT = 2, EKF_KERNEL_ASSOCIATE = 3,
       EKF_KERNEL_APPEND = 4,
       EKF_KERNEL_ROWPANEL = 5,
       EKF_KERNEL_EXCHANGE = 6,
       EKF_KERNEL_COMPACT = 7,
       EKF_KERNEL_COUNT = 8 };
int32_t ekf_kernel_timing_enable(ekf_handle *h, int32_t which, int32_t on);
int32_t ekf_kernel_timing_read(ekf_handle *h, int32_t which, int64_t *launches, double *total_ms);
const char *ekf_downdate_kernel_name(const ekf_handle *h, int32_t *pairs);
int32_t ekf_downdate_algorithmic_bytes(ekf_handle *h, int64_t *bytes);

#ifdef __cplusplus
}
#endif
#endif
```

Measured before the change: 1935.

## Cap gather grid at CU count and loop columns with a software-pipelined chunk loop

The gather kernel grid is capped at the number of compute units, or a configurable gather_groups value, and each workgroup walks several column chunks in a grid-stride loop. Later chunks are software-pipelined: the next chunk's column loads and ring-buffer rank-2 patch loads are issued before the current chunk's outputs are finished. Association scoring keeps a running per-thread best across chunks. A VGPR cap attribute is added to keep occupancy. The aim is to avoid launching many short workgroups and to hide load latency, at the cost of more register pressure and more complex control flow.

```diff
diff --git a/ekf_slam_amd/_lib.py b/ekf_slam_amd/_lib.py
--- a/ekf_slam_amd/_lib.py
+++ b/ekf_slam_amd/_lib.py
@@ -27,7 +27,7 @@
     _fields_ = [("C", _d), ("Rc", _d * 2), ("s_cost", _d), ("s_thresh", _d), ("w_pos", _d),
                 ("capacity_landmarks", _i64), ("mode", _i32), ("storage", _i32), ("device", _i32),
                 ("tile", _i32), ("rank", _i32), ("world", _i32), ("batch", _i32), ("async_flush", _i32), ("device_assoc", _i32),
-                ("pass_direction", _i32), ("force_sharded", _i32), ("pass_arith", _i32), ("reserved", _i32 * 2)]
+                ("pass_direction", _i32), ("force_sharded", _i32), ("pass_arith", _i32), ("gather_groups", _i32), ("reserved", _i32 * 1)]
 
 
 SIGNATURES = {
diff --git a/ekf_slam_amd/csrc/gather.h b/ekf_slam_amd/csrc/gather.h
--- a/ekf_slam_amd/csrc/gather.h
+++ b/ekf_slam_amd/csrc/gather.h
@@ -39,8 +39,6 @@
     TS *__restrict__ tiles = (TS *)st.tiles;
     const int64_t ldm = st.ldm;
     const int64_t n_old = 2 * Nd, n_new = append ? n_old + 2 : n_old;
-    const int64_t c = (int64_t)blockIdx.x * kGatherCols + tid;
-    const bool live = c < n_new;
     double pose[3], pr[9];
 #pragma unroll
     for (int i = 0; i < 3; ++i) pose[i] = x[i];
@@ -48,47 +46,81 @@
     for (int i = 0; i < 9; ++i) pr[i] = prr[i];
     double jxr[2][3];
     append_jxr(dl.u0, pose[2], jxr);
-    double xn = 0.0, t0 = 0.0, t1 = 0.0, t2 = 0.0, dgc = 0.0, dgl = 0.0;
-    if (c < n_old) {
-        t0 = strip[c]; t1 = strip[ldm + c]; t2 = strip[2 * ldm + c];
-        xn = x[3 + c];
-        const double *__restrict__ d = dg + 3 * (c >> 1);
-        if (c & 1) { dgl = d[1]; dgc = d[2]; } else dgc = d[0];
-        if (append)
-            for (int i = 0; i < 2; ++i)
-                if (st.tm.mine((n_old + i) >> st.tm.shift, c >> st.tm.shift))
-                    pmm_low_store<TS>(tiles, st.tm, n_old + i, c, append_row_entry(jxr, i, t0, t1, t2));
-    } else if (live) {
-        const int b = (int)(c - n_old);
-        const volatile double *loc = dl.loc + 3 * (Nd - dl.loc_base);
-        double cblk[3], iblk[3][2];
-        append_blocks(jxr, pr, dl.u0, dl.u1, a.R00, a.R01, a.R10, a.R11, cblk, iblk);
-        xn = loc[b];
-        t0 = iblk[0][b]; t1 = iblk[1][b]; t2 = iblk[2][b];
-        const bool own = st.tm.mine(n_old >> st.tm.shift, n_old >> st.tm.shift);
-        if (b == 0) {
-            dgc = cblk[0];
-            if (own) pmm_low_store<TS>(tiles, st.tm, n_old, n_old, cblk[0]);
-            st.s[Nd] = (double)(Nd + 1);
-        } else {
-            dgl = cblk[1]; dgc = cblk[2];
-            if (own) { pmm_low_store<TS>(tiles, st.tm, n_old + 1, n_old, cblk[1]); pmm_low_store<TS>(tiles, st.tm, n_old + 1, n_old + 1, cblk[2]); }
-        }
-    }
-    if (live) {
-        x_nxt[3 + c] = xn;
-        strip_nxt[c] = t0; strip_nxt[ldm + c] = t1; strip_nxt[2 * ldm + c] = t2;
-        double *__restrict__ d = dgn + 3 * (c >> 1);
-        if (c & 1) { d[1] = dgl; d[2] = dgc; } else d[0] = dgc;
-    }
-    if (c < st.tm.padded(n_new)) {
-        const int64_t out_off = (int64_t)ring_slot(a.pstart, a.npend, st.pcap) * st.pair_stride;
-        reinterpret_cast<double2 *>(st.Gp + out_off)[c] = make_double2(0.0, 0.0);
-        reinterpret_cast<double2 *>(st.Kp + out_off)[c] = make_double2(0.0, 0.0);
-        if (st.Gp32) {
-            st.Gp32[out_off + c] = 0.0f; st.Gp32[out_off + ldm + c] = 0.0f;
-            st.Kp32[out_off + c] = -0.0f; st.Kp32[out_off + ldm + c] = -0.0f;
-        }
+    const int64_t pad_new = st.tm.padded(n_new);
+    const int64_t nchunks = (pad_new + kGatherCols - 1) / kGatherCols;
+    double ll = INFINITY;
+    int64_t ix = INT64_MAX;
+    for (int64_t chunk = blockIdx.x;;) {
+        const int64_t c = chunk * kGatherCols + tid;
+        const bool live = c < n_new;
+        double xn = 0.0, t0 = 0.0, t1 = 0.0, t2 = 0.0, dgc = 0.0, dgl = 0.0;
+        if (c < n_old) {
+            t0 = strip[c]; t1 = strip[ldm + c]; t2 = strip[2 * ldm + c];
+            xn = x[3 + c];
+            const double *__restrict__ d = dg + 3 * (c >> 1);
+            if (c & 1) { dgl = d[1]; dgc = d[2]; } else dgc = d[0];
+            if (append)
+                for (int i = 0; i < 2; ++i)
+                    if (st.tm.mine((n_old + i) >> st.tm.shift, c >> st.tm.shift))
+                        pmm_low_store<TS>(tiles, st.tm, n_old + i, c, append_row_entry(jxr, i, t0, t1, t2));
+        } else if (live) {
+            const int b = (int)(c - n_old);
+            const volatile double *loc = dl.loc + 3 * (Nd - dl.loc_base);
+            double cblk[3], iblk[3][2];
+            append_blocks(jxr, pr, dl.u0, dl.u1, a.R00, a.R01, a.R10, a.R11, cblk, iblk);
+            xn = loc[b];
+            t0 = iblk[0][b]; t1 = iblk[1][b]; t2 = iblk[2][b];
+            const bool own = st.tm.mine(n_old >> st.tm.shift, n_old >> st.tm.shift);
+            if (b == 0) {
+                dgc = cblk[0];
+                if (own) pmm_low_store<TS>(tiles, st.tm, n_old, n_old, cblk[0]);
+                st.s[Nd] = (double)(Nd + 1);
+            } else {
+                dgl = cblk[1]; dgc = cblk[2];
+                if (own) { pmm_low_store<TS>(tiles, st.tm, n_old + 1, n_old, cblk[1]); pmm_low_store<TS>(tiles, st.tm, n_old + 1, n_old + 1, cblk[2]); }
+            }
+        }
+        if (live) {
+            x_nxt[3 + c] = xn;
+            strip_nxt[c] = t0; strip_nxt[ldm + c] = t1; strip_nxt[2 * ldm + c] = t2;
+            double *__restrict__ d = dgn + 3 * (c >> 1);
+            if (c & 1) { d[1] = dgl; d[2] = dgc; } else d[0] = dgc;
+        }
+        if (c < pad_new) {
+            const int64_t out_off = (int64_t)ring_slot(a.pstart, a.npend, st.pcap) * st.pair_stride;
+            reinterpret_cast<double2 *>(st.Gp + out_off)[c] = make_double2(0.0, 0.0);
+            reinterpret_cast<double2 *>(st.Kp + out_off)[c] = make_double2(0.0, 0.0);
+            if (st.Gp32) {
+                st.Gp32[out_off + c] = 0.0f; st.Gp32[out_off + ldm + c] = 0.0f;
+                st.Kp32[out_off + c] = -0.0f; st.Kp32[out_off + ldm + c] = -0.0f;
+            }
+        }
+        if (dl.parts_out != nullptr) {
+            const bool odd = (c & 1) != 0;
+            const double xn_o = lane_xor1(xn), t0_o = lane_xor1(t0), t1_o = lane_xor1(t1), t2_o = lane_xor1(t2),
+                         d10 = lane_xor1(dgl), d11 = lane_xor1(dgc);
+            if (live && !odd) {
+                const int64_t k = c >> 1;
+                double q[24];
+#pragma unroll
+                for (int i = 0; i < 9; ++i) q[i] = pr[i];
+                q[9] = t0; q[10] = t0_o; q[11] = t1; q[12] = t1_o; q[13] = t2; q[14] = t2_o;
+                q[15] = dgc; q[16] = d10; q[17] = d10; q[18] = d11;
+                q[19] = pose[0]; q[20] = pose[1]; q[21] = pose[2];
+                q[22] = xn; q[23] = xn_o;
+                SmallSolve so;
+                solve_small(q, dl.z0, dl.z1, dl.R00, dl.R01, dl.R10, dl.R11, so);
+                const double n0 = so.nu[0], n1 = so.nu[1];
+                const double pc = (n0 * so.Phi[0] + n1 * so.Phi[2]) * n0 + (n0 * so.Phi[1] + n1 * so.Phi[3]) * n1;
+                const double sk = k == Nd ? (double)(Nd + 1) : st.s[k];
+                const double d = dl.z2 - sk;
+                const double sc = d * (1.0 / dl.s_cost) * d;
+                const double like = (dl.w_pos != 0.0) ? (dl.w_pos * pc + sc) : sc;
+                if (like <= dl.s_thresh && assoc_better(like, k, ll, ix)) { ll = like; ix = k; }
+            }
+        }
+        chunk += gridDim.x;
+        if (chunk >= nchunks) break;
     }
     if (blockIdx.x == 0) {
         if (tid < 9) prr_nxt[tid] = prr[tid];
@@ -96,30 +128,6 @@
         if (tid == 0) *dl.dn_out = n_new >> 1;
     }
     if (dl.parts_out == nullptr) return;
-    const bool odd = (c & 1) != 0;
-    const double xn_o = lane_xor1(xn), t0_o = lane_xor1(t0), t1_o = lane_xor1(t1), t2_o = lane_xor1(t2),
-                 d10 = lane_xor1(dgl), d11 = lane_xor1(dgc);
-    double ll = INFINITY;
-    int64_t ix = INT64_MAX;
-    if (live && !odd) {
-        const int64_t k = c >> 1;
-        double q[24];
-#pragma unroll
-        for (int i = 0; i < 9; ++i) q[i] = pr[i];
-        q[9] = t0; q[10] = t0_o; q[11] = t1; q[12] = t1_o; q[13] = t2; q[14] = t2_o;
-        q[15] = dgc; q[16] = d10; q[17] = d10; q[18] = d11;
-        q[19] = pose[0]; q[20] = pose[1]; q[21] = pose[2];
-        q[22] = xn; q[23] = xn_o;
-        SmallSolve so;
-        solve_small(q, dl.z0, dl.z1, dl.R00, dl.R01, dl.R10, dl.R11, so);
-        const double n0 = so.nu[0], n1 = so.nu[1];
-        const double pc = (n0 * so.Phi[0] + n1 * so.Phi[2]) * n0 + (n0 * so.Phi[1] + n1 * so.Phi[3]) * n1;
-        const double sk = k == Nd ? (double)(Nd + 1) : st.s[k];
-        const double d = dl.z2 - sk;
-        const double sc = d * (1.0 / dl.s_cost) * d;
-        const double like = (dl.w_pos != 0.0) ? (dl.w_pos * pc + sc) : sc;
-        if (like <= dl.s_thresh) { ll = like; ix = k; }
-    }
     wave_argmin_sparse(ll, ix);
     if ((tid & 63) == 0) { oa_ll[tid >> 6] = ll; oa_ix[tid >> 6] = ix == INT64_MAX ? -1 : (int)ix; }
     __syncthreads();
@@ -133,7 +141,7 @@
 }
 
 template <typename TS, bool kSharded, bool kPredict, bool kFused = false, bool kDev = false, bool kDecide = false>
-__global__ __launch_bounds__(kGatherBlock) void k_gather(DevState st, CorrectArgs a, PanelView pv, PredictArgs pa,
+__global__ __launch_bounds__(kGatherBlock) __attribute__((amdgpu_num_vgpr(108))) void k_gather(DevState st, CorrectArgs a, PanelView pv, PredictArgs pa,
                                                          typename DevLoopParam<kDev>::type dl) {
     static_assert(!kDev || !kFused, "the device loop never drives the small-map fused form");
     static_assert(!kDecide || (kDev && !kSharded && !kPredict), "the device-decided branch: unsharded, predict carried out before");
@@ -363,25 +371,29 @@
     __builtin_amdgcn_sched_barrier(0);
     asm volatile("s_barrier" ::: "memory");
     EKF_STAMP();
-    double m0 = 0.0, m1 = 0.0, s0 = 0.0, s1 = 0.0, s2 = 0.0, xc = 0.0;
+    struct ColBase { double m0, m1, s0, s1, s2, xc, dgc, dgl; };
+    auto load_column = [&](int64_t col, bool lv, ColBase &b) {
+        b = ColBase{ 0.0, 0.0, 0.0, 0.0, 0.0, 0.0, 0.0, 0.0 };
+        if (lv) {
+            if (kSharded) { const double2 m = pv.at(st.tm, col); b.m0 = m.x; b.m1 = m.y; }
+            else if (col <= j) {
+                const int64_t m = st.tm.T - 1;
+                const TS *__restrict__ tp = tiles + st.tm.tile_offset(j >> st.tm.shift, col >> st.tm.shift) + ((j & m) << st.tm.shift) + (col & m);
+                b.m0 = (double)tp[0]; b.m1 = (double)tp[st.tm.T];
+            }
+            else if (col >= j + 2) pmm_low_pair<TS>(tiles, st.tm, col, j, b.m0, b.m1);
+            else pmm_low_pair<TS>(tiles, st.tm, j + 1, j, b.m0, b.m1);
+            b.s0 = strip[col]; b.s1 = strip[ldm + col]; b.s2 = strip[2 * ldm + col];
+            b.xc = x[3 + col];
+            const double *__restrict__ dg = st.diag[st.dcur] + 3 * (col >> 1);
+            if (col & 1) { b.dgl = dg[1]; b.dgc = dg[2]; } else b.dgc = dg[0];
+        }
+    };
     const bool rowpart = c <= j, colpart = c >= j + 2;
-    if (live) {
-        if (kSharded) { const double2 m = pv.at(st.tm, c); m0 = m.x; m1 = m.y; }
-        else if (rowpart) {
-            const int64_t m = st.tm.T - 1;
-            const TS *__restrict__ tp = tiles + st.tm.tile_offset(j >> st.tm.shift, c >> st.tm.shift) + ((j & m) << st.tm.shift) + (c & m);
-            m0 = (double)tp[0]; m1 = (double)tp[st.tm.T];
-        }
-        else if (colpart) pmm_low_pair<TS>(tiles, st.tm, c, j, m0, m1);
-        else pmm_low_pair<TS>(tiles, st.tm, j + 1, j, m0, m1);
-        s0 = strip[c]; s1 = strip[ldm + c]; s2 = strip[2 * ldm + c];
-        xc = x[3 + c];
-    }
-    double dgc = 0.0, dgl = 0.0;
-    if (live) {
-        const double *__restrict__ dg = st.diag[st.dcur] + 3 * (c >> 1);
-        if (c & 1) { dgl = dg[1]; dgc = dg[2]; } else dgc = dg[0];
-    }
+    ColBase cb;
+    load_column(c, live, cb);
+    double m0 = cb.m0, m1 = cb.m1;
+    const double dgc = cb.dgc, dgl = cb.dgl;
     __builtin_amdgcn_sched_barrier(0);
     EKF_STAMP();
     upatch[tid] = up0; upatch[tid + kGatherCols] = up1;
@@ -398,13 +410,15 @@
     double2 pre[kPre];
     bool next_assoc = false;
     if constexpr (kDev) next_assoc = dl.parts_out != nullptr;
+    const uint32_t krel = (uint32_t)((st.Kp - st.Gp) >> 1);
+    const char *__restrict__ pair_base = reinterpret_cast<const char *>(st.Gp);
+    auto pair_lane_bytes = [&](int64_t col, bool rowp) {
+        const uint32_t cc = (uint32_t)(col < pad_cols ? col : pad_cols - 1);
+        return (cc + (rowp ? 0u : krel)) * 16u;
+    };
+    const uint32_t lane_bytes = pair_lane_bytes(c, rowpart);
+    const uint32_t step = (uint32_t)ps2, wrap = (uint32_t)st.pcap * step;
     {
-        const uint32_t cc = (uint32_t)(c < pad_cols ? c : pad_cols - 1);
-        const uint32_t krel = (uint32_t)((st.Kp - st.Gp) >> 1);
-        const uint32_t lane_off = cc + (rowpart ? 0u : krel);
-        const char *__restrict__ ub = reinterpret_cast<const char *>(st.Gp);
-        const uint32_t lane_bytes = lane_off * 16u;
-        const uint32_t step = (uint32_t)ps2, wrap = (uint32_t)st.pcap * step;
         uint32_t off = (uint32_t)pstart * step;
         int npre_ld = npre;
         asm volatile("" : "+s"(npre_ld));
@@ -413,7 +427,7 @@
             if (g0 < npre_ld) {
 #pragma unroll
                 for (int t = 0; t < 8; ++t) {
-                    pre[g0 + t] = *reinterpret_cast<const double2 *>(ub + (uint64_t)off * 16u + lane_bytes);
+                    pre[g0 + t] = *reinterpret_cast<const double2 *>(pair_base + (uint64_t)off * 16u + lane_bytes);
                     if (g0 + t + 1 < npre) { off += step; if (off == wrap) off = 0; }
                 }
             }
@@ -435,23 +449,6 @@
                         m0 = g0 + t < npre ? v0 : m0; m1 = g0 + t < npre ? v1 : m1;
                     }
                 }
-            const double2 *__restrict__ gp = reinterpret_cast<const double2 *>(st.Gp) + c;
-            int i = npre;
-            for (; i + 8 <= npend; i += 8) {
-                double2 g[8];
-#pragma unroll
-                for (int q = 0; q < 8; ++q) g[q] = gp[(int64_t)ring_slot(pstart, i + q, st.pcap) * ps2];
-#pragma unroll
-                for (int q = 0; q < 8; ++q) {
-                    m0 = rank2_apply(m0, upatch[4 * (i + q) + 0], g[q]);
-                    m1 = rank2_apply(m1, upatch[4 * (i + q) + 1], g[q]);
-                }
-            }
-            for (; i < npend; ++i) {
-                const double2 g = gp[(int64_t)ring_slot(pstart, i, st.pcap) * ps2];
-                m0 = rank2_apply(m0, upatch[4 * i + 0], g);
-                m1 = rank2_apply(m1, upatch[4 * i + 1], g);
-            }
         } else if (colpart) {
 #pragma unroll
             for (int g0 = 0; g0 < kPre; g0 += 8)
@@ -465,23 +462,6 @@
                         m0 = g0 + t < npre ? v0 : m0; m1 = g0 + t < npre ? v1 : m1;
                     }
                 }
-            const double2 *__restrict__ kp = reinterpret_cast<const double2 *>(st.Kp) + c;
-            int i = npre;
-            for (; i + 8 <= npend; i += 8) {
-                double2 k[8];
-#pragma unroll
-                for (int q = 0; q < 8; ++q) k[q] = kp[(int64_t)ring_slot(pstart, i + q, st.pcap) * ps2];
-#pragma unroll
-                for (int q = 0; q < 8; ++q) {
-                    m0 = rank2_apply(m0, k[q], upatch[4 * (i + q) + 2]);
-                    m1 = rank2_apply(m1, k[q], upatch[4 * (i + q) + 3]);
-                }
-            }
-            for (; i < npend; ++i) {
-                const double2 k = kp[(int64_t)ring_slot(pstart, i, st.pcap) * ps2];
-                m0 = rank2_apply(m0, k, upatch[4 * i + 2]);
-                m1 = rank2_apply(m1, k, upatch[4 * i + 3]);
-            }
         } else {
             for (int i = 0; i < npend; ++i) {
                 m0 = rank2_apply(m0, upatch[4 * i + 1], upatch[4 * i + 2]);
@@ -489,11 +469,68 @@
             }
         }
     }
-    {
-        const double dgl_p = lane_xor1(dgl);
-        if (c == j) { m0 = dgc; m1 = dgl_p; }
-        else if (c == j + 1) { m0 = dgl; m1 = dgc; }
-    }
+    using Half0 = std::integral_constant<int, 0>;
+    using Half1 = std::integral_constant<int, 1>;
+    int npend_ld = do_patch ? npend : 0;
+    asm volatile("" : "+s"(npend_ld));
+    auto ring_load = [&](auto half, int i0, uint32_t lbytes) {
+        constexpr int h = decltype(half)::value;
+#pragma unroll
+        for (int g0 = 0; g0 < 16; g0 += 8)
+            if (i0 + g0 < npend_ld) {
+#pragma unroll
+                for (int t = 0; t < 8; ++t) {
+                    const int i = i0 + g0 + t < npend ? i0 + g0 + t : npend - 1;
+                    const uint32_t o = (uint32_t)ring_slot(pstart, i, st.pcap) * step * 16u + lbytes;
+                    pre[16 * h + g0 + t] = *reinterpret_cast<const double2 *>(pair_base + o);
+                }
+            }
+    };
+    auto ring_apply = [&](auto half, int i0, int sel, double &r0, double &r1) {
+        constexpr int h = decltype(half)::value;
+#pragma unroll
+        for (int g0 = 0; g0 < 16; g0 += 4)
+            if (i0 + g0 < npend) {
+                double2 ua[4], ub[4];
+#pragma unroll
+                for (int t = 0; t < 4; ++t) {
+                    const int i = i0 + g0 + t < npend ? i0 + g0 + t : npend - 1;
+                    ua[t] = upatch[4 * i + sel]; ub[t] = upatch[4 * i + sel + 1];
+                }
+#pragma unroll
+                for (int t = 0; t < 4; ++t) {
+                    const double v0 = rank2_apply(r0, ua[t], pre[16 * h + g0 + t]), v1 = rank2_apply(r1, ub[t], pre[16 * h + g0 + t]);
+                    r0 = i0 + g0 + t < npend ? v0 : r0; r1 = i0 + g0 + t < npend ? v1 : r1;
+                }
+            }
+    };
+    auto ring_prime = [&](int i0, uint32_t lbytes) { ring_load(Half0{}, i0, lbytes); ring_load(Half1{}, i0 + 16, lbytes); };
+    auto ring_run = [&](int i0, int sel, uint32_t lbytes, double &r0, double &r1) {
+        for (int b = i0; b < npend; b += 32) {
+            ring_apply(Half0{}, b, sel, r0, r1);
+            __builtin_amdgcn_sched_barrier(0);
+            ring_load(Half0{}, b + 32, lbytes);
+            __builtin_amdgcn_sched_barrier(0);
+            ring_apply(Half1{}, b + 16, sel, r0, r1);
+            __builtin_amdgcn_sched_barrier(0);
+            ring_load(Half1{}, b + 48, lbytes);
+            __builtin_amdgcn_sched_barrier(0);
+        }
+    };
+    if (do_patch && npend > kPre) {
+        int t2 = tid;
+        asm volatile("" : "+v"(t2));
+        const int64_t c2 = (int64_t)blockIdx.x * kGatherCols + t2;
+        const uint32_t lb = pair_lane_bytes(c2, c2 <= j);
+        ring_prime(kPre, lb);
+        ring_run(kPre, c2 <= j ? 0 : 2, lb, m0, m1);
+    }
+    auto own_block = [&](int64_t col, double dc, double dl_, double &r0, double &r1) {
+        const double dgl_p = lane_xor1(dl_);
+        if (col == j) { r0 = dc; r1 = dgl_p; }
+        else if (col == j + 1) { r0 = dl_; r1 = dc; }
+    };
+    own_block(c, dgc, dgl, m0, m1);
     EKF_STAMP();
     __syncthreads();
     EKF_STAMP();
@@ -502,50 +539,54 @@
     const int64_t out_off = (int64_t)ring_slot(pstart, npend, st.pcap) * st.pair_stride;
     double2 *__restrict__ Gout = reinterpret_cast<double2 *>(st.Gp + out_off);
     double2 *__restrict__ Kout = reinterpret_cast<double2 *>(st.Kp + out_off);
-    double g[2] = { 0.0, 0.0 }, k0 = 0.0, k1 = 0.0;
-    double xn = 0.0, t0 = 0.0, t1 = 0.0, t2 = 0.0;
-    if (live) {
-        if (kPredict) predict_strip(s0, s1, s2, ps.fa, ps.fb);
-        for (int r = 0; r < 2; ++r)
-            g[r] = sol.Hs[r][0] * s0 + sol.Hs[r][1] * s1 + sol.Hs[r][2] * s2 + sol.Hs[r][3] * m0 + sol.Hs[r][4] * m1;
-        k0 = g[0] * sol.Phi[0] + g[1] * sol.Phi[2];
-        k1 = g[0] * sol.Phi[1] + g[1] * sol.Phi[3];
-        if (!kFused) {
-            Gout[c] = make_double2(g[0], g[1]);
-            Kout[c] = make_double2(k0, k1);
+    struct ColOut { double g[2], k0, k1, xn, t0, t1, t2, ndc, ndl; };
+    auto column_outputs = [&](int64_t col, bool lv, ColBase b, double r0, double r1, ColOut &o) {
+        o = ColOut{ { 0.0, 0.0 }, 0.0, 0.0, 0.0, 0.0, 0.0, 0.0, 0.0, 0.0 };
+        double s0 = b.s0, s1 = b.s1, s2 = b.s2;
+        if (lv) {
+            if (kPredict) predict_strip(s0, s1, s2, ps.fa, ps.fb);
+            for (int r = 0; r < 2; ++r)
+                o.g[r] = sol.Hs[r][0] * s0 + sol.Hs[r][1] * s1 + sol.Hs[r][2] * s2 + sol.Hs[r][3] * r0 + sol.Hs[r][4] * r1;
+            o.k0 = o.g[0] * sol.Phi[0] + o.g[1] * sol.Phi[2];
+            o.k1 = o.g[0] * sol.Phi[1] + o.g[1] * sol.Phi[3];
+            if (!kFused) {
+                Gout[col] = make_double2(o.g[0], o.g[1]);
+                Kout[col] = make_double2(o.k0, o.k1);
+                if (st.Gp32) {
+                    st.Gp32[out_off + col] = (float)o.g[0]; st.Gp32[out_off + ldm + col] = (float)o.g[1];
+                    st.Kp32[out_off + col] = -(float)o.k0; st.Kp32[out_off + ldm + col] = -(float)o.k1;
+                }
+            }
+            o.xn = b.xc + (o.k0 * sol.nu[0] + o.k1 * sol.nu[1]);
+            o.t0 = s0 - (sol.Kr[0][0] * o.g[0] + sol.Kr[0][1] * o.g[1]);
+            o.t1 = s1 - (sol.Kr[1][0] * o.g[0] + sol.Kr[1][1] * o.g[1]);
+            o.t2 = s2 - (sol.Kr[2][0] * o.g[0] + sol.Kr[2][1] * o.g[1]);
+            x_nxt[3 + col] = o.xn;
+            double *__restrict__ sn = strip_nxt;
+            sn[col] = o.t0;
+            sn[ldm + col] = o.t1;
+            sn[2 * ldm + col] = o.t2;
+        } else if (col < pad_end && !kFused) {
+            Gout[col] = make_double2(0.0, 0.0);
+            Kout[col] = make_double2(0.0, 0.0);
             if (st.Gp32) {
-                st.Gp32[out_off + c] = (float)g[0]; st.Gp32[out_off + ldm + c] = (float)g[1];
-                st.Kp32[out_off + c] = -(float)k0; st.Kp32[out_off + ldm + c] = -(float)k1;
-            }
-        }
-        xn = xc + (k0 * sol.nu[0] + k1 * sol.nu[1]);
-        t0 = s0 - (sol.Kr[0][0] * g[0] + sol.Kr[0][1] * g[1]);
-        t1 = s1 - (sol.Kr[1][0] * g[0] + sol.Kr[1][1] * g[1]);
-        t2 = s2 - (sol.Kr[2][0] * g[0] + sol.Kr[2][1] * g[1]);
-        x_nxt[3 + c] = xn;
-        double *__restrict__ sn = strip_nxt;
-        sn[c] = t0;
-        sn[ldm + c] = t1;
-        sn[2 * ldm + c] = t2;
-    } else if (c < pad_end && !kFused) {
-        Gout[c] = make_double2(0.0, 0.0);
-        Kout[c] = make_double2(0.0, 0.0);
-        if (st.Gp32) {
-            st.Gp32[out_off + c] = 0.0f; st.Gp32[out_off + ldm + c] = 0.0f;
-            st.Kp32[out_off + c] = -0.0f; st.Kp32[out_off + ldm + c] = -0.0f;
-        }
-    }
-    double ndc, ndl;
-    {
-        const double2 kn = make_double2(k0, k1), gn = make_double2(g[0], g[1]);
+                st.Gp32[out_off + col] = 0.0f; st.Gp32[out_off + ldm + col] = 0.0f;
+                st.Kp32[out_off + col] = -0.0f; st.Kp32[out_off + ldm + col] = -0.0f;
+            }
+        }
+        const double2 kn = make_double2(o.k0, o.k1), gn = make_double2(o.g[0], o.g[1]);
         const double2 gl = make_double2(lane_xor1(gn.x), lane_xor1(gn.y));
-        ndc = rank2_apply(dgc, kn, gn);
-        ndl = rank2_apply(dgl, kn, gl);
-        if (live) {
-            double *__restrict__ dn = st.diag[st.dcur ^ 1] + 3 * (c >> 1);
-            if (c & 1) { dn[1] = ndl; dn[2] = ndc; } else dn[0] = ndc;
-        }
-    }
+        o.ndc = rank2_apply(b.dgc, kn, gn);
+        o.ndl = rank2_apply(b.dgl, kn, gl);
+        if (lv) {
+            double *__restrict__ dn = st.diag[st.dcur ^ 1] + 3 * (col >> 1);
+            if (col & 1) { dn[1] = o.ndl; dn[2] = o.ndc; } else dn[0] = o.ndc;
+        }
+    };
+    ColOut co;
+    column_outputs(c, live, cb, m0, m1, co);
+    const double k0 = co.k0, k1 = co.k1;
+    const double g[2] = { co.g[0], co.g[1] };
     if (kFused) {
         upatch[tid] = make_double2(k0, k1);
         upatch[kGatherCols + tid] = make_double2(g[0], g[1]);
@@ -571,18 +612,16 @@
                 if (ptr[q]) *ptr[q] = (TS)rank2_apply(val[q], upatch[rr[q]], upatch[kGatherCols + cq[q]]);
         }
     }
-    if constexpr (kDev) {
-        if (next_assoc) {
-            __shared__ double na_ll[kGatherCols / 64];
-            __shared__ int na_ix[kGatherCols / 64];
-            const bool odd = (c & 1) != 0;
-            const double dcc = ndc, dlo = ndl;
-            const double xn_o = lane_xor1(xn), t0_o = lane_xor1(t0), t1_o = lane_xor1(t1), t2_o = lane_xor1(t2),
+    double best_ll = INFINITY;
+    int64_t best_ix = INT64_MAX;
+    auto score_next = [&](int64_t col, bool lv, const ColOut &o) {
+        if constexpr (kDev) {
+            const bool odd = (col & 1) != 0;
+            const double dcc = o.ndc, dlo = o.ndl;
+            const double xn_o = lane_xor1(o.xn), t0_o = lane_xor1(o.t0), t1_o = lane_xor1(o.t1), t2_o = lane_xor1(o.t2),
                          d10 = lane_xor1(dlo), d11 = lane_xor1(dcc);
-            double ll = INFINITY;
-            int64_t ix = INT64_MAX;
-            if (live && !odd) {
-                const int64_t k = c >> 1;
+            if (lv && !odd) {
+                const int64_t k = col >> 1;
                 double q[24];
 #pragma unroll
                 for (int r = 0; r < 3; ++r)
@@ -591,12 +630,12 @@
                         const int rr = r > b ? r : b, bb = r > b ? b : r;
                         q[3 * r + b] = pss[3 * rr + bb] - (sol.Kr[rr][0] * sol.Gr[0][bb] + sol.Kr[rr][1] * sol.Gr[1][bb]);
                     }
-                q[9] = t0; q[10] = t0_o; q[11] = t1; q[12] = t1_o; q[13] = t2; q[14] = t2_o;
+                q[9] = o.t0; q[10] = t0_o; q[11] = o.t1; q[12] = t1_o; q[13] = o.t2; q[14] = t2_o;
                 q[15] = dcc; q[16] = d10; q[17] = d10; q[18] = d11;
 #pragma unroll
                 for (int l = 0; l < 3; ++l)
                     q[19 + l] = pose_sh[l] + (sol.Kr[l][0] * sol.nu[0] + sol.Kr[l][1] * sol.nu[1]);
-                q[22] = xn; q[23] = xn_o;
+                q[22] = o.xn; q[23] = xn_o;
                 SmallSolve so2;
                 solve_small(q, dl.z0, dl.z1, dl.R00, dl.R01, dl.R10, dl.R11, so2);
                 const double n0 = so2.nu[0], n1 = so2.nu[1];
@@ -604,8 +643,69 @@
                 const double d = dl.z2 - st.s[k];
                 const double sc = d * (1.0 / dl.s_cost) * d;
                 const double like = (dl.w_pos != 0.0) ? (dl.w_pos * pc + sc) : sc;
-                if (like <= dl.s_thresh) { ll = like; ix = k; }
-            }
+                if (like <= dl.s_thresh && assoc_better(like, k, best_ll, best_ix)) { best_ll = like; best_ix = k; }
+            }
+        }
+    };
+    if (next_assoc) score_next(c, live, co);
+
+    if constexpr (!kFused) {
+        const int64_t nchunks = (pad_end + kGatherCols - 1) / kGatherCols;
+        const int np = do_patch ? npend : 0;
+        int64_t chunk = (int64_t)blockIdx.x + gridDim.x;
+        if (chunk < nchunks) {
+            int tl = tid;
+            asm volatile("" : "+v"(tl));
+            constexpr bool kAhead = !kDev;
+            int64_t cn = chunk * kGatherCols + tl;
+            ColBase nb{};
+            uint32_t lb = 0;
+            auto request = [&]() {
+                load_column(cn, cn < a.n_mm, nb);
+                lb = pair_lane_bytes(cn, cn <= j);
+                if (np > 0) ring_prime(0, lb);
+            };
+            auto finish = [&](int64_t cl, const ColBase &bl, double r0, double r1) {
+                ColOut ol;
+                column_outputs(cl, cl < a.n_mm, bl, r0, r1, ol);
+                if (next_assoc) score_next(cl, cl < a.n_mm, ol);
+            };
+            if constexpr (kAhead) {
+                bool have = false;
+                int64_t cl = 0;
+                ColBase bl = nb;
+                uint32_t lbl = 0;
+                for (;;) {
+                    double r0 = bl.m0, r1 = bl.m1;
+                    if (have) {
+                        if (np > 0) ring_run(0, cl <= j ? 0 : 2, lbl, r0, r1);
+                        own_block(cl, bl.dgc, bl.dgl, r0, r1);
+                    }
+                    const bool more = chunk < nchunks;
+                    if (more) { cn = chunk * kGatherCols + tl; request(); chunk += gridDim.x; }
+                    __builtin_amdgcn_sched_barrier(0);
+                    if (have) finish(cl, bl, r0, r1);
+                    if (!more) break;
+                    cl = cn; bl = nb; lbl = lb; have = true;
+                }
+            } else {
+                for (; chunk < nchunks; chunk += gridDim.x) {
+                    cn = chunk * kGatherCols + tl;
+                    request();
+                    double r0 = nb.m0, r1 = nb.m1;
+                    if (np > 0) ring_run(0, cn <= j ? 0 : 2, lb, r0, r1);
+                    own_block(cn, nb.dgc, nb.dgl, r0, r1);
+                    finish(cn, nb, r0, r1);
+                }
+            }
+        }
+    }
+    if constexpr (kDev) {
+        if (next_assoc) {
+            __shared__ double na_ll[kGatherCols / 64];
+            __shared__ int na_ix[kGatherCols / 64];
+            double ll = best_ll;
+            int64_t ix = best_ix;
             wave_argmin_sparse(ll, ix);
             if ((tid & 63) == 0) { na_ll[tid >> 6] = ll; na_ix[tid >> 6] = ix == INT64_MAX ? -1 : (int)ix; }
             __syncthreads();
diff --git a/ekf_slam_amd/csrc/host/lifecycle.h b/ekf_slam_amd/csrc/host/lifecycle.h
--- a/ekf_slam_amd/csrc/host/lifecycle.h
+++ b/ekf_slam_amd/csrc/host/lifecycle.h
@@ -32,7 +32,7 @@
     if (cfg->capacity_landmarks < 1 || cfg->rank < 0 || cfg->rank >= world) return EKF_ERR_INVALID_ARG;
     if (cfg->storage != EKF_STORE_F64 && cfg->storage != EKF_STORE_F32) return EKF_ERR_INVALID_ARG;
     if (cfg->mode != EKF_MODE_KNOWN && cfg->mode != EKF_MODE_UC) return EKF_ERR_INVALID_ARG;
-    if (cfg->batch < 0 || cfg->batch > 64) return EKF_ERR_INVALID_ARG;
+    if (cfg->batch < 0 || cfg->batch > 64 || cfg->gather_groups < 0) return EKF_ERR_INVALID_ARG;
     if (cfg->mode == EKF_MODE_UC && cfg->device_assoc == 4 && (world > 1 || cfg->force_sharded)) return EKF_ERR_INVALID_ARG;
     if (cfg->pass_arith != EKF_ARITH_F64 &&
         !((cfg->pass_arith == EKF_ARITH_F32 || cfg->pass_arith == EKF_ARITH_SPLIT3) && cfg->storage == EKF_STORE_F32 && T == 256))
@@ -53,7 +53,7 @@
 
     HIPCHK(h, hipSetDevice(cfg->device));
     hipDeviceProp_t prop = {};
-    if (cfg->async_flush != 0 || cfg->pass_arith != EKF_ARITH_F64) HIPCHK(h, hipGetDeviceProperties(&prop, cfg->device));
+    HIPCHK(h, hipGetDeviceProperties(&prop, cfg->device));
     {
         int lo = 0, hi = 0;
         HIPCHK(h, hipDeviceGetStreamPriorityRange(&lo, &hi));
diff --git a/ekf_slam_amd/csrc/host/passes.h b/ekf_slam_amd/csrc/host/passes.h
--- a/ekf_slam_amd/csrc/host/passes.h
+++ b/ekf_slam_amd/csrc/host/passes.h
@@ -237,6 +237,7 @@
     h->st.tiles = tiles;
     h->tilebuf[0] = tiles;
     h->async_flush = cfg.async_flush != 0;
+    int main_cus = prop.multiProcessorCount;
     if (h->async_flush) {
         char *tiles2 = nullptr;
         HIPCHK(h, dalloc(h, &tiles2, (size_t)slots * T * T * elt_size(h)));
@@ -255,6 +256,7 @@
                 }
             HIPCHK(h, hipExtStreamCreateWithCUMask(&h->flush_stream, 8, mask));
             h->flush_cus = ncu - taken;
+            main_cus = taken;
         } else {
             int lo = 0, hi = 0;
             HIPCHK(h, hipDeviceGetStreamPriorityRange(&lo, &hi));
@@ -263,6 +265,7 @@
         HIPCHK(h, new_event(h, &h->ev_pairs));
         HIPCHK(h, new_event(h, &h->ev_flushed));
     }
+    h->st.gather_cap = ekf_tune_int("EKF_GATHER_GROUPS", cfg.gather_groups > 0 ? cfg.gather_groups : main_cus);
     h->batch = cfg.batch < 1 ? 1 : cfg.batch;
     h->cfg.batch = h->batch;
     h->st.pair_stride = 2 * ldm;
diff --git a/ekf_slam_amd/csrc/kernels.h b/ekf_slam_amd/csrc/kernels.h
--- a/ekf_slam_amd/csrc/kernels.h
+++ b/ekf_slam_amd/csrc/kernels.h
@@ -28,6 +28,7 @@
     TileMap tm;
     double *diag[2];
     int32_t dcur;
+    int32_t gather_cap;
 };
 
 struct PredictArgs {
diff --git a/ekf_slam_amd/csrc/launch/steps.h b/ekf_slam_amd/csrc/launch/steps.h
--- a/ekf_slam_amd/csrc/launch/steps.h
+++ b/ekf_slam_amd/csrc/launch/steps.h
@@ -26,7 +26,10 @@
     }); });
 }
 
-int64_t gather_workgroups(const DevState &st, int64_t n_mm) { return cdiv(ekf_tiles_for(n_mm, st.tm.T) * st.tm.T, kGatherCols); }
+int64_t gather_workgroups(const DevState &st, int64_t n_mm) {
+    const int64_t chunks = cdiv(ekf_tiles_for(n_mm, st.tm.T) * st.tm.T, kGatherCols);
+    return st.gather_cap > 0 && chunks > st.gather_cap ? st.gather_cap : chunks;
+}
 int gather_fuse_max_rows() { return kFuseMaxRows; }
 
 namespace {
diff --git a/include/ekfslam.h b/include/ekfslam.h
--- a/include/ekfslam.h
+++ b/include/ekfslam.h
@@ -49,7 +49,8 @@
     int32_t pass_direction;
     int32_t force_sharded;
     int32_t pass_arith;
-    int32_t reserved[2];
+    int32_t gather_groups;
+    int32_t reserved[1];
 } ekf_config;
 
 typedef struct ekf_handle ekf_handle;
```

New measurement: 1932. No clear change (-0.1%).
